# henintsoa98/srsRAN_4G

Hardware: AMD Instinct MI355X
Metric: turbo-decoded info Mbps + PDSCH subframes/s, 20 MHz 64QAM, 1/2/4/8 GPU (higher is better)
Workload: dtype int16; 1 GPU; tdec all 188 LTE CB sizes x 1024 CBs, 8 half-its, rm_turbo SB layout; cb_sizes=188, parallelism=cb-sharded x1, tdec16=auto

## Files before the change

include/srsran_tdec.h:

```cpp
#ifndef SRSRAN_AMD_TDEC_H
#define SRSRAN_AMD_TDEC_H

#include <stdbool.h>
#include <stdint.h>

#ifdef __cplusplus
extern "C" {
#endif

#ifndef SRSRAN_SUCCESS
#define SRSRAN_SUCCESS 0
#define SRSRAN_ERROR -1
#define SRSRAN_ERROR_INVALID_INPUTS -2
#endif

#define SRSRAN_TCOD_RATE 3
#define SRSRAN_TCOD_TOTALTAIL 12
#define SRSRAN_TCOD_MAX_LEN_CB 6144
#define SRSRAN_TDEC_EXPECT_INPUT_SB 1
#define SRSRAN_NOF_TC_CB_SIZES 188

typedef enum {
  SRSRAN_TDEC_AUTO = 0,
  SRSRAN_TDEC_GENERIC,
  SRSRAN_TDEC_SSE,
  SRSRAN_TDEC_SSE_WINDOW,
  SRSRAN_TDEC_NEON_WINDOW,
  SRSRAN_TDEC_AVX_WINDOW,
  SRSRAN_TDEC_SSE8_WINDOW,
  SRSRAN_TDEC_AVX8_WINDOW,
  SRSRAN_TDEC_NOF_IMP
} srsran_tdec_impl_type_t;

typedef struct {
  uint32_t                max_long_cb;
  bool                    force_not_sb;
  srsran_tdec_impl_type_t dec_type;
  uint32_t                current_long_cb;
  int                     current_cbidx;
  int                     n_iter;
  void*                   gpu;
} srsran_tdec_t;

int srsran_tdec_init(srsran_tdec_t* h, uint32_t max_long_cb);
int srsran_tdec_init_manual(srsran_tdec_t* h, uint32_t max_long_cb, srsran_tdec_impl_type_t dec_type);
void srsran_tdec_free(srsran_tdec_t* h);
void srsran_tdec_force_not_sb(srsran_tdec_t* h);
int srsran_tdec_new_cb(srsran_tdec_t* h, uint32_t long_cb);
int srsran_tdec_get_nof_iterations(srsran_tdec_t* h);
uint32_t srsran_tdec_autoimp_get_subblocks(uint32_t long_cb);
uint32_t srsran_tdec_autoimp_get_subblocks_8bit(uint32_t long_cb);
void srsran_tdec_iteration(srsran_tdec_t* h, int16_t* input, uint8_t* output);
int srsran_tdec_run_all(srsran_tdec_t* h, int16_t* input, uint8_t* output, uint32_t nof_iterations, uint32_t long_cb);
void srsran_tdec_iteration_8bit(srsran_tdec_t* h, int8_t* input, uint8_t* output);
int  srsran_tdec_run_all_8bit(srsran_tdec_t* h, int8_t* input, uint8_t* output, uint32_t nof_iterations, uint32_t long_cb);

int srsran_tdec_gpu_run_batch_8bit(uint32_t      long_cb,
                                   const int8_t* d_input,
                                   uint32_t      in_stride,
                                   int           layout_sb,
                                   uint8_t*      d_output,
                                   uint32_t      nof_cb,
                                   uint32_t      nof_iterations,
                                   void*         stream);

int srsran_tdec_run_all_batch(srsran_tdec_t* h,
                              const int16_t* input,
                              uint32_t       in_stride,
                              uint8_t*       output,
                              uint32_t       nof_cb,
                              uint32_t       nof_iterations,
                              uint32_t       long_cb);

int srsran_tdec_gpu_run_batch(uint32_t       long_cb,
                              const int16_t* d_input,
                              uint32_t       in_stride,
                              int            layout_sb,
                              uint8_t*       d_output,
                              uint32_t       nof_cb,
                              uint32_t       nof_iterations,
                              void*          stream);

int srsran_tdec_gpu_run_multi(uint32_t              nof_groups,
                              const uint32_t*       long_cb,
                              const int16_t* const* d_input,
                              const uint32_t*       in_stride,
                              int                   layout_sb,
                              uint8_t* const*       d_output,
                              const uint32_t*       nof_cb,
                              uint32_t              nof_iterations,
                              void*                 stream);

int srsran_tdec_gpu_available(void);

const char* srsran_tdec_gpu_kernel_name(uint32_t long_cb);

const char* srsran_tdec_gpu_kernel_name_batch(uint32_t long_cb, uint32_t nof_cb);

const char* srsran_tdec_gpu_last_kernel(void);

void     srsran_tdec_gpu_set_pair_threshold(uint32_t nof_cb);
uint32_t srsran_tdec_gpu_get_pair_threshold(void);
void     srsran_tdec_gpu_set_class_single_threshold(uint32_t nof_subblocks, uint32_t nof_cb);
uint32_t srsran_tdec_gpu_get_class_single_threshold(uint32_t nof_subblocks);
void     srsran_tdec_gpu_set_single_threshold(uint32_t nof_cb);
uint32_t srsran_tdec_gpu_get_single_threshold(void);
void     srsran_tdec_gpu_set_generic_single_threshold(uint32_t nof_cb);
void     srsran_tdec_gpu_set_w8_max_k(uint32_t k);
uint32_t srsran_tdec_gpu_get_w8_max_k(void);
void     srsran_tdec_gpu_set_w8_fused_max_k(uint32_t k);
uint32_t srsran_tdec_gpu_get_w8_fused_max_k(void);
uint32_t srsran_tdec_gpu_get_generic_single_threshold(void);

#ifdef __cplusplus
}
#endif
#endif
```

srsran_4g_amd/csrc/tdec_api.cpp:

```cpp
#include <hip/hip_runtime.h>

#include <cstdio>
#include <cstdlib>
#include <algorithm>
#include <cstring>
#include <map>
#include <tuple>
#include <mutex>
#include <vector>

#include "../../include/srsran_tdec.h"
#include "stage_copy.h"
#include "devkey.h"
#include "tdec_kernel.h"
#include "tdec8bit_kernel.h"

using namespace srsran_amd;

namespace {

const uint16_t kCbSizes[SRSRAN_NOF_TC_CB_SIZES] = {
    40,   48,   56,   64,   72,   80,   88,   96,   104,  112,  120,  128,  136,  144,  152,  160,  168,  176,  184,
    192,  200,  208,  216,  224,  232,  240,  248,  256,  264,  272,  280,  288,  296,  304,  312,  320,  328,  336,
    344,  352,  360,  368,  376,  384,  392,  400,  408,  416,  424,  432,  440,  448,  456,  464,  472,  480,  488,
    496,  504,  512,  528,  544,  560,  576,  592,  608,  624,  640,  656,  672,  688,  704,  720,  736,  752,  768,
    784,  800,  816,  832,  848,  864,  880,  896,  912,  928,  944,  960,  976,  992,  1008, 1024, 1056, 1088, 1120,
    1152, 1184, 1216, 1248, 1280, 1312, 1344, 1376, 1408, 1440, 1472, 1504, 1536, 1568, 1600, 1632, 1664, 1696, 1728,
    1760, 1792, 1824, 1856, 1888, 1920, 1952, 1984, 2016, 2048, 2112, 2176, 2240, 2304, 2368, 2432, 2496, 2560, 2624,
    2688, 2752, 2816, 2880, 2944, 3008, 3072, 3136, 3200, 3264, 3328, 3392, 3456, 3520, 3584, 3648, 3712, 3776, 3840,
    3904, 3968, 4032, 4096, 4160, 4224, 4288, 4352, 4416, 4480, 4544, 4608, 4672, 4736, 4800, 4864, 4928, 4992, 5056,
    5120, 5184, 5248, 5312, 5376, 5440, 5504, 5568, 5632, 5696, 5760, 5824, 5888, 5952, 6016, 6080, 6144};

const uint16_t kF1[SRSRAN_NOF_TC_CB_SIZES] = {
    3,   7,   19,  7,   7,   11,  5,   11,  7,   41,  103, 15,  9,   17,  9,   21,  101, 21,  57, 23,  13,
    27,  11,  27,  85,  29,  33,  15,  17,  33,  103, 19,  19,  37,  19,  21,  21,  115, 193, 21, 133, 81,
    45,  23,  243, 151, 155, 25,  51,  47,  91,  29,  29,  247, 29,  89,  91,  157, 55,  31,  17, 35,  227,
    65,  19,  37,  41,  39,  185, 43,  21,  155, 79,  139, 23,  217, 25,  17,  127, 25,  239, 17, 137, 215,
    29,  15,  147, 29,  59,  65,  55,  31,  17,  171, 67,  35,  19,  39,  19,  199, 21,  211, 21, 43,  149,
    45,  49,  71,  13,  17,  25,  183, 55,  127, 27,  29,  29,  57,  45,  31,  59,  185, 113, 31, 17,  171,
    209, 253, 367, 265, 181, 39,  27,  127, 143, 43,  29,  45,  157, 47,  13,  111, 443, 51,  51, 451, 257,
    57,  313, 271, 179, 331, 363, 375, 127, 31,  33,  43,  33,  477, 35,  233, 357, 337, 37,  71, 71,  37,
    39,  127, 39,  39,  31,  113, 41,  251, 43,  21,  43,  45,  45,  161, 89,  323, 47,  23,  47, 263};
const uint16_t kF2[SRSRAN_NOF_TC_CB_SIZES] = {
    10,  12,  42,  16,  18,  20,  22,  24,  26,  84,  90,  32,  34,  108, 38,  120, 84,  44,  46,  48,  50,
    52,  36,  56,  58,  60,  62,  32,  198, 68,  210, 36,  74,  76,  78,  120, 82,  84,  86,  44,  90,  46,
    94,  48,  98,  40,  102, 52,  106, 72,  110, 168, 114, 58,  118, 180, 122, 62,  84,  64,  66,  68,  420,
    96,  74,  76,  234, 80,  82,  252, 86,  44,  120, 92,  94,  48,  98,  80,  102, 52,  106, 48,  110, 112,
    114, 58,  118, 60,  122, 124, 84,  64,  66,  204, 140, 72,  74,  76,  78,  240, 82,  252, 86,  88,  60,
    92,  846, 48,  28,  80,  102, 104, 954, 96,  110, 112, 114, 116, 354, 120, 610, 124, 420, 64,  66,  136,
    420, 216, 444, 456, 468, 80,  164, 504, 172, 88,  300, 92,  188, 96,  28,  240, 204, 104, 212, 192, 220,
    336, 228, 232, 236, 120, 244, 248, 168, 64,  130, 264, 134, 408, 138, 280, 142, 480, 146, 444, 120, 152,
    462, 234, 158, 80,  96,  902, 166, 336, 170, 86,  174, 176, 178, 120, 182, 184, 186, 94,  190, 480};

int cb_index(uint32_t K)
{
  for (int i = 0; i < SRSRAN_NOF_TC_CB_SIZES; i++) {
    if (kCbSizes[i] == K) {
      return i;
    }
  }
  return -1;
}

constexpr size_t kMaxLds = 160 * 1024;

struct Config {
  int       nsb;
  TdecArgs  proto;
  uint16_t* d_tfwd = nullptr;
  uint16_t* d_trev = nullptr;
  uint16_t* d_tfwd_nat = nullptr;
  uint16_t* d_trev_nat = nullptr;
};

std::mutex                             g_mu;
std::map<std::tuple<int, uint32_t, int>, Config*> g_cfg;
int                                    g_have_gpu = -1;

bool have_gpu()
{
  if (g_have_gpu < 0) {
    int n = 0;
    g_have_gpu = (hipGetDeviceCount(&n) == hipSuccess && n > 0) ? 1 : 0;
  }
  return g_have_gpu == 1;
}

Config* get_config(uint32_t K, int nsb)
{
  std::lock_guard<std::mutex> lk(g_mu);
  auto key = std::make_tuple(cur_dev(), K, nsb);
  auto it  = g_cfg.find(key);
  if (it != g_cfg.end()) {
    return it->second;
  }
  const int idx = cb_index(K);
  if (idx < 0 || !have_gpu()) {
    return nullptr;
  }
  TdecArgs a{};
  a.K = K;
  if (nsb > 1) {
    if (K % nsb || K / nsb < (uint32_t)TDEC_OVERLAP) {
      return nullptr;
    }
    a.L   = K / nsb;
    a.Ls  = a.L | 1u;
    a.xyw = nsb * a.Ls;
    a.M   = (a.L + TDEC_W - 1) / TDEC_W;
  } else {
    a.L   = K;
    a.Ls  = (K + 3) | 1u;
    a.xyw = a.Ls;
    a.M   = (K + 3 + TDEC_W - 1) / TDEC_W;
  }
  a.magicL  = (uint32_t)(((1ull << 32) + a.L - 1) / a.L);
  a.magicLs = (uint32_t)(((1ull << 32) + a.Ls - 1) / a.Ls);
  if (tdec_lds_bytes(nsb, a.xyw, a.M) > kMaxLds) {
    return nullptr;
  }
  std::vector<uint16_t> fwd(K), rev(K), tf(K), tr(K), tfn(K), trn(K);
  const uint64_t f1 = kF1[idx], f2 = kF2[idx];
  for (uint64_t i = 0; i < K; i++) {
    const uint32_t j = (uint32_t)((f1 * i + f2 * i * i) % K);
    fwd[i]           = (uint16_t)j;
    rev[j]           = (uint16_t)i;
  }
  auto slot = [&](uint32_t n) -> uint16_t {
    return nsb > 1 ? (uint16_t)((n / a.L) * a.Ls + n % a.L) : (uint16_t)n;
  };
  for (uint32_t q = 0; q < K; q++) {
    const uint32_t n = nsb > 1 ? (q % nsb) * a.L + q / nsb : q;
    tf[q]            = slot(fwd[n]);
    tr[q]            = slot(rev[n]);
    tfn[q]           = slot(fwd[q]);
    trn[q]           = slot(rev[q]);
  }
  Config* c = new Config();
  c->nsb    = nsb;
  c->proto  = a;
  auto up = [&](uint16_t** d, const std::vector<uint16_t>& h) {
    return hipMalloc(d, K * sizeof(uint16_t)) == hipSuccess &&
           hipMemcpy(*d, h.data(), K * sizeof(uint16_t), hipMemcpyHostToDevice) == hipSuccess;
  };
  if (!up(&c->d_tfwd, tf) || !up(&c->d_trev, tr) || !up(&c->d_tfwd_nat, tfn) || !up(&c->d_trev_nat, trn)) {
    fprintf(stderr, "[srsran_tdec] device table allocation failed for K=%u\n", K);
    delete c;
    return nullptr;
  }
  g_cfg[key] = c;
  return c;
}

int auto_nsb(uint32_t K)
{
  const uint32_t n = srsran_tdec_autoimp_get_subblocks(K);
  return n ? (int)n : 1;
}

int nsb_for(const srsran_tdec_t* h, uint32_t K)
{
  switch (h->dec_type) {
    case SRSRAN_TDEC_AUTO:
      return auto_nsb(K);
    case SRSRAN_TDEC_GENERIC:
      return 1;
    case SRSRAN_TDEC_SSE_WINDOW:
      return 8;
    case SRSRAN_TDEC_AVX_WINDOW:
      return 16;
    default:
      return -1;
  }
}

struct Ctx {
  hipStream_t stream = nullptr;
  short*      d_in   = nullptr;
  uint8_t*    d_out  = nullptr;
  short*      d_state = nullptr;
  size_t      state_elems = 0;
  short*      d_bin  = nullptr;
  uint8_t*    d_bout = nullptr;
  size_t      bin_elems = 0, bout_bytes = 0;
};

const size_t kMaxIn = 3 * (SRSRAN_TCOD_MAX_LEN_CB + 32) + SRSRAN_TCOD_TOTALTAIL;

int enqueue(const Config* c, const short* d_in, uint32_t in_stride, int layout_sb, uint8_t* d_out, uint32_t ncb,
            int n_start, int n_end, short* d_state, hipStream_t stream)
{
  TdecArgs a  = c->proto;
  a.in        = d_in;
  a.in_stride = in_stride;
  a.layout_sb = (c->nsb > 1) ? layout_sb : 0;
  a.ncb       = ncb;
  a.n_start   = n_start;
  a.n_end     = n_end;
  a.out       = d_out;
  a.tfwd      = c->d_tfwd;
  a.trev      = c->d_trev;
  a.tfwd_nat  = c->d_tfwd_nat;
  a.trev_nat  = c->d_trev_nat;
  a.state     = d_state;
  hipError_t e = tdec_launch(c->nsb, a, stream);
  if (e != hipSuccess) {
    fprintf(stderr, "[srsran_tdec] launch failed: %s\n", hipGetErrorString(e));
    return SRSRAN_ERROR;
  }
  return SRSRAN_SUCCESS;
}

bool grow(void** p, size_t* have, size_t need)
{
  if (*have >= need) {
    return true;
  }
  if (*p) {
    (void)hipFree(*p);
    *p = nullptr;
  }
  if (hipMalloc(p, need) != hipSuccess) {
    *have = 0;
    return false;
  }
  *have = need;
  return true;
}

struct XpowTables {
  const uint32_t* d[2] = {nullptr, nullptr};
};
std::map<int, XpowTables> g_xpow;

const XpowTables* xpow_tables()
{
  std::lock_guard<std::mutex> lk(g_mu);
  const int dev = cur_dev();
  auto      it  = g_xpow.find(dev);
  if (it != g_xpow.end()) {
    return &it->second;
  }
  const int             nm = SRSRAN_TCOD_MAX_LEN_CB / 8 + 1;
  std::vector<uint32_t> h(nm);
  uint32_t*             d[2] = {nullptr, nullptr};
  const uint32_t        poly[2] = {LTE_CRC24A, LTE_CRC24B};
  for (int i = 0; i < 2; i++) {
    crc24_xpow_table(poly[i], h.data(), nm);
    if (hipMalloc(&d[i], nm * sizeof(uint32_t)) != hipSuccess ||
        hipMemcpy(d[i], h.data(), nm * sizeof(uint32_t), hipMemcpyHostToDevice) != hipSuccess) {
      return nullptr;
    }
  }
  XpowTables& t = g_xpow[dev];
  t.d[0]        = d[0];
  t.d[1]        = d[1];
  return &t;
}

std::map<std::pair<int, uint32_t>, const uint16_t*> g_qpp8;

const uint16_t* qpp8_table(uint32_t K, uint32_t nsb, int idx)
{
  std::lock_guard<std::mutex> lk(g_mu);
  const auto                  key = std::make_pair(cur_dev(), K);
  auto                        it  = g_qpp8.find(key);
  if (it != g_qpp8.end()) {
    return it->second;
  }
  const uint64_t        f1 = kF1[idx], f2 = kF2[idx], Ls = K / nsb;
  std::vector<uint16_t> h(K);
  for (uint64_t j = 0; j < K; j++) {
    const uint64_t n  = (j % nsb) * Ls + j / nsb;
    const uint64_t fn = ((f2 * n % K) * n + f1 * n) % K;
    h[j]              = (uint16_t)((fn % Ls) * nsb + fn / Ls);
  }
  uint16_t* d = nullptr;
  if (hipMalloc((void**)&d, K * sizeof(uint16_t)) != hipSuccess ||
      hipMemcpy(d, h.data(), K * sizeof(uint16_t), hipMemcpyHostToDevice) != hipSuccess) {
    hipFree(d);
    return nullptr;
  }
  g_qpp8[key] = d;
  return d;
}

}

namespace srsran_amd {
void qpp_coeffs(uint32_t idx, uint32_t* f1, uint32_t* f2)
{
  *f1 = kF1[idx];
  *f2 = kF2[idx];
}
}

namespace srsran_amd {

int tdec_cb_index(uint32_t K) { return cb_index(K); }

int tdec_sch_enqueue(uint32_t      K,
                     const TdecCb* d_cbs,
                     uint32_t      ncb,
                     uint8_t*      d_out,
                     uint32_t      out_stride,
                     uint8_t*      d_noi,
                     uint8_t*      d_crc_ok,
                     int           n_end,
                     hipStream_t   stream)
{
  if (ncb == 0) {
    return SRSRAN_SUCCESS;
  }
  Config* c = get_config(K, auto_nsb(K));
  const XpowTables* xp = xpow_tables();
  if (!c || !xp) {
    return SRSRAN_ERROR;
  }
  TdecArgs a   = c->proto;
  a.in         = nullptr;
  a.in_stride  = 0;
  a.layout_sb  = c->nsb > 1 ? 1 : 0;
  a.ncb        = ncb;
  a.n_start    = 0;
  a.n_end      = n_end > 0 ? n_end : 1;
  a.out        = d_out;
  a.tfwd       = c->d_tfwd;
  a.trev       = c->d_trev;
  a.tfwd_nat   = c->d_tfwd_nat;
  a.trev_nat   = c->d_trev_nat;
  a.state      = nullptr;
  a.cbs        = d_cbs;
  a.out_stride = out_stride;
  a.noi_out    = d_noi;
  a.crc_ok     = d_crc_ok;
  a.xpow_a     = xp->d[0];
  a.xpow_b     = xp->d[1];
  a.min_iters  = 2;
  hipError_t e = tdec_launch(c->nsb, a, stream);
  if (e != hipSuccess) {
    fprintf(stderr, "[srsran_sch] turbo launch failed: %s\n", hipGetErrorString(e));
    return SRSRAN_ERROR;
  }
  return SRSRAN_SUCCESS;
}

}

namespace {
struct Scratch8 {
  void*       p = nullptr;
  hipStream_t s = nullptr;
  Scratch8(hipStream_t stream, size_t bytes) : s(stream)
  {
    if (hipMallocAsync(&p, bytes, stream) != hipSuccess) {
      p = nullptr;
    }
  }
  ~Scratch8()
  {
    if (p) {
      hipFreeAsync(p, s);
    }
  }
  Scratch8(const Scratch8&)            = delete;
  Scratch8& operator=(const Scratch8&) = delete;
};
}

namespace srsran_amd {
int tdec8_sch_enqueue(uint32_t      K,
                      const TdecCb* d_cbs,
                      uint32_t      ncb,
                      uint8_t*      d_out,
                      uint32_t      out_stride,
                      uint8_t*      d_noi,
                      uint8_t*      d_crc_ok,
                      int           n_end,
                      hipStream_t   stream)
{
  if (ncb == 0) {
    return SRSRAN_SUCCESS;
  }
  const int      idx = cb_index(K);
  const uint32_t nsb = srsran_tdec_autoimp_get_subblocks_8bit(K);
  const XpowTables* xp = xpow_tables();
  if (idx < 0 || (nsb != 16 && nsb != 32) || !xp) {
    return SRSRAN_ERROR;
  }
  Tdec8Args a{};
  a.in         = nullptr;
  a.layout_sb  = 1;
  a.K          = K;
  a.ncb        = ncb;
  a.n_end      = n_end > 0 ? n_end : 1;
  a.out        = d_out;
  a.cbs        = d_cbs;
  a.out_stride = out_stride;
  a.noi_out    = d_noi;
  a.crc_ok     = d_crc_ok;
  a.xpow_a     = xp->d[0];
  a.xpow_b     = xp->d[1];
  a.min_iters  = 2;
  a.qpp        = qpp8_table(K, nsb, idx);
  if (!a.qpp) {
    return SRSRAN_ERROR;
  }
  Scratch8 beta(stream, tdec8bit_beta_bytes((int)nsb, K, ncb));
  a.beta = (uint2*)beta.p;
  if (!a.beta) {
    return SRSRAN_ERROR;
  }
  const hipError_t e = tdec8bit_launch((int)nsb, a, stream);
  tdec_set_last_kernel(nsb == 32 ? "tdec8bit_kernel<32>" : "tdec8bit_kernel<16>");
  if (e != hipSuccess) {
    fprintf(stderr, "[srsran_sch] 8-bit turbo launch failed: %s\n", hipGetErrorString(e));
    return SRSRAN_ERROR;
  }
  return SRSRAN_SUCCESS;
}
}

extern "C" {

uint32_t srsran_tdec_autoimp_get_subblocks(uint32_t long_cb)
{
  if (!(long_cb % 16) && long_cb > 800) {
    return 16;
  }
  if (!(long_cb % 8) && long_cb > 400) {
    return 8;
  }
  return 0;
}

uint32_t srsran_tdec_autoimp_get_subblocks_8bit(uint32_t long_cb)
{
  if (!(long_cb % 32) && long_cb > 2048) {
    return 32;
  }
  if (!(long_cb % 16) && long_cb > 800) {
    return 16;
  }
  if (!(long_cb % 8) && long_cb > 400) {
    return 8;
  }
  return 0;
}

int srsran_tdec_gpu_available(void)
{
  std::lock_guard<std::mutex> lk(g_mu);
  return have_gpu() ? 1 : 0;
}

const char* srsran_tdec_gpu_kernel_name(uint32_t long_cb)
{
  switch (auto_nsb(long_cb)) {
    case 16:
      return "tdec_kernel<16>";
    case 8:
      return "tdec_kernel<8>";
    default:
      return "tdec_kernel<1>";
  }
}

const char* srsran_tdec_gpu_last_kernel(void) { return tdec_last_kernel(); }

void srsran_tdec_gpu_set_pair_threshold(uint32_t nof_cb) { tdec16_set_min_cb(nof_cb); }

uint32_t srsran_tdec_gpu_get_pair_threshold(void) { return tdec16_min_cb(); }

void srsran_tdec_gpu_set_w8_max_k(uint32_t k) { tdecs_set_w8_max_k(k); }

uint32_t srsran_tdec_gpu_get_w8_max_k(void) { return tdecs_w8_max_k(); }

void srsran_tdec_gpu_set_w8_fused_max_k(uint32_t k) { tdecs_set_w8_fused_max_k(k); }

uint32_t srsran_tdec_gpu_get_w8_fused_max_k(void) { return tdecs_w8_fused_max_k(); }



void srsran_tdec_gpu_set_class_single_threshold(uint32_t nof_subblocks, uint32_t nof_cb)
{
  if (nof_subblocks == 16) {
    tdec16s_set_min_cb(nof_cb);
  } else if (nof_subblocks == 8) {
    tdec8s_set_min_cb(nof_cb);
  } else if (nof_subblocks <= 1) {
    tdec1s_set_min_cb(nof_cb);
  }
}

uint32_t srsran_tdec_gpu_get_class_single_threshold(uint32_t nof_subblocks)
{
  return nof_subblocks == 16 ? tdec16s_min_cb() : nof_subblocks == 8 ? tdec8s_min_cb() : tdec1s_min_cb();
}

void srsran_tdec_gpu_set_single_threshold(uint32_t nof_cb)
{
  tdec16s_set_min_cb(nof_cb);
  tdec8s_set_min_cb(nof_cb);
}

uint32_t srsran_tdec_gpu_get_single_threshold(void) { return tdec16s_min_cb(); }

void srsran_tdec_gpu_set_generic_single_threshold(uint32_t nof_cb) { tdec1s_set_min_cb(nof_cb); }

uint32_t srsran_tdec_gpu_get_generic_single_threshold(void) { return tdec1s_min_cb(); }

const char* srsran_tdec_gpu_kernel_name_batch(uint32_t long_cb, uint32_t nof_cb)
{
  const int nsb = auto_nsb(long_cb);
  if (nsb == 16) {
    const int k = tdec16_choice(nof_cb);
    if (k) {
      return k == 2 ? "tdec16s_kernel" : "tdec16_kernel";
    }
  }
  if (nsb == 8 && nof_cb >= tdec8s_min_cb()) {
    return "tdec8s_kernel";
  }
  if (nsb == 1 && nof_cb >= tdec1s_min_cb()) {
    return "tdec1s_kernel";
  }
  return srsran_tdec_gpu_kernel_name(long_cb);
}

int srsran_tdec_init(srsran_tdec_t* h, uint32_t max_long_cb)
{
  return srsran_tdec_init_manual(h, max_long_cb, SRSRAN_TDEC_AUTO);
}

int srsran_tdec_init_manual(srsran_tdec_t* h, uint32_t max_long_cb, srsran_tdec_impl_type_t dec_type)
{
  if (!h) {
    return SRSRAN_ERROR_INVALID_INPUTS;
  }
  memset(h, 0, sizeof(*h));
  if (dec_type != SRSRAN_TDEC_AUTO && dec_type != SRSRAN_TDEC_GENERIC && dec_type != SRSRAN_TDEC_SSE_WINDOW &&
      dec_type != SRSRAN_TDEC_AVX_WINDOW) {
    fprintf(stderr, "[srsran_tdec] decoder %d not supported\n", (int)dec_type);
    return SRSRAN_ERROR;
  }
  if (max_long_cb > SRSRAN_TCOD_MAX_LEN_CB) {
    return SRSRAN_ERROR;
  }
  {
    std::lock_guard<std::mutex> lk(g_mu);
    if (!have_gpu()) {
      fprintf(stderr, "[srsran_tdec] no HIP device available\n");
      return SRSRAN_ERROR;
    }
  }
  Ctx* c = new Ctx();
  if (hipStreamCreateWithFlags(&c->stream, hipStreamNonBlocking) != hipSuccess ||
      hipMalloc(&c->d_in, kMaxIn * sizeof(short)) != hipSuccess ||
      hipMalloc(&c->d_out, SRSRAN_TCOD_MAX_LEN_CB / 8) != hipSuccess) {
    delete c;
    return SRSRAN_ERROR;
  }
  hipMemset(c->d_in, 0, kMaxIn * sizeof(short));
  h->gpu           = c;
  h->max_long_cb   = max_long_cb;
  h->dec_type      = dec_type;
  h->current_cbidx = -1;
  return SRSRAN_SUCCESS;
}

void srsran_tdec_free(srsran_tdec_t* h)
{
  if (!h) {
    return;
  }
  Ctx* c = (Ctx*)h->gpu;
  if (c) {
    if (c->stream) {
      hipStreamSynchronize(c->stream);
      hipStreamDestroy(c->stream);
    }
    hipFree(c->d_in);
    hipFree(c->d_out);
    hipFree(c->d_state);
    hipFree(c->d_bin);
    hipFree(c->d_bout);
    delete c;
  }
  memset(h, 0, sizeof(*h));
}

void srsran_tdec_force_not_sb(srsran_tdec_t* h)
{
  if (h) {
    h->force_not_sb = true;
  }
}

int srsran_tdec_new_cb(srsran_tdec_t* h, uint32_t long_cb)
{
  if (!h || long_cb > h->max_long_cb) {
    fprintf(stderr, "[srsran_tdec] TDEC was initialized for max_long_cb=%d\n", h ? h->max_long_cb : 0);
    return SRSRAN_ERROR;
  }
  h->n_iter          = 0;
  h->current_long_cb = long_cb;
  h->current_cbidx   = cb_index(long_cb);
  if (h->current_cbidx < 0) {
    fprintf(stderr, "[srsran_tdec] Invalid CB length %d\n", long_cb);
    return SRSRAN_ERROR;
  }
  return SRSRAN_SUCCESS;
}

int srsran_tdec_get_nof_iterations(srsran_tdec_t* h) { return h ? h->n_iter : 0; }

static size_t input_len(const srsran_tdec_t* h, const Config* c, uint32_t K)
{
  const bool sb = !h->force_not_sb && c->nsb > 1;
  return sb ? 3 * (K + 32) + 12 : 3 * K + 12;
}

void srsran_tdec_iteration(srsran_tdec_t* h, int16_t* input, uint8_t* output)
{
  if (!h || !h->gpu || h->current_cbidx < 0) {
    fprintf(stderr, "[srsran_tdec] Error CB index not set (call srsran_tdec_new_cb() first\n");
    return;
  }
  Ctx*           ctx = (Ctx*)h->gpu;
  const uint32_t K   = h->current_long_cb;
  Config*        c   = get_config(K, nsb_for(h, K));
  if (!c) {
    fprintf(stderr, "[srsran_tdec] unsupported K=%u\n", K);
    return;
  }
  const size_t st = 2 * (size_t)c->proto.xyw;
  if (!grow((void**)&ctx->d_state, &ctx->state_elems, st * sizeof(short))) {
    return;
  }
  if (h->n_iter == 0) {
    hipMemcpyAsync(ctx->d_in, input, input_len(h, c, K) * sizeof(short), hipMemcpyHostToDevice, ctx->stream);
  }
  if (enqueue(c, ctx->d_in, (uint32_t)kMaxIn, !h->force_not_sb, ctx->d_out, 1, h->n_iter, h->n_iter + 1,
              ctx->d_state, ctx->stream)) {
    return;
  }
  hipMemcpyAsync(output, ctx->d_out, K / 8, hipMemcpyDeviceToHost, ctx->stream);
  hipStreamSynchronize(ctx->stream);
  h->n_iter++;
}

int srsran_tdec_run_all(srsran_tdec_t* h, int16_t* input, uint8_t* output, uint32_t nof_iterations, uint32_t long_cb)
{
  if (srsran_tdec_new_cb(h, long_cb)) {
    return SRSRAN_ERROR;
  }
  int ret = srsran_tdec_run_all_batch(h, input, 0, output, 1, nof_iterations, long_cb);
  if (ret == SRSRAN_SUCCESS) {
    h->n_iter = nof_iterations > 0 ? (int)nof_iterations : 1;
  }
  return ret;
}

int srsran_tdec_run_all_batch(srsran_tdec_t* h,
                              const int16_t* input,
                              uint32_t       in_stride,
                              uint8_t*       output,
                              uint32_t       nof_cb,
                              uint32_t       nof_iterations,
                              uint32_t       long_cb)
{
  if (!h || !h->gpu || !input || !output) {
    return SRSRAN_ERROR_INVALID_INPUTS;
  }
  if (long_cb > h->max_long_cb || cb_index(long_cb) < 0) {
    return SRSRAN_ERROR;
  }
  if (nof_cb == 0) {
    return SRSRAN_SUCCESS;
  }
  Ctx*    ctx = (Ctx*)h->gpu;
  Config* c   = get_config(long_cb, nsb_for(h, long_cb));
  if (!c) {
    return SRSRAN_ERROR;
  }
  const size_t len = input_len(h, c, long_cb);
  if (in_stride == 0) {
    in_stride = (uint32_t)len;
  }
  if (in_stride < len) {
    return SRSRAN_ERROR_INVALID_INPUTS;
  }
  const size_t in_elems  = (size_t)in_stride * (nof_cb - 1) + len;
  const size_t out_bytes = (size_t)nof_cb * (long_cb / 8);
  if (!grow((void**)&ctx->d_bin, &ctx->bin_elems, in_elems * sizeof(short)) ||
      !grow((void**)&ctx->d_bout, &ctx->bout_bytes, out_bytes)) {
    return SRSRAN_ERROR;
  }
  hipMemcpyAsync(ctx->d_bin, input, in_elems * sizeof(short), hipMemcpyHostToDevice, ctx->stream);
  const int n_end = nof_iterations > 0 ? (int)nof_iterations : 1;
  if (enqueue(c, ctx->d_bin, in_stride, !h->force_not_sb, ctx->d_bout, nof_cb, 0, n_end, nullptr, ctx->stream)) {
    return SRSRAN_ERROR;
  }
  hipMemcpyAsync(output, ctx->d_bout, out_bytes, hipMemcpyDeviceToHost, ctx->stream);
  if (hipStreamSynchronize(ctx->stream) != hipSuccess) {
    fprintf(stderr, "[srsran_tdec] decode failed: %s\n", hipGetErrorString(hipGetLastError()));
    return SRSRAN_ERROR;
  }
  return SRSRAN_SUCCESS;
}

int srsran_tdec_gpu_run_batch(uint32_t       long_cb,
                              const int16_t* d_input,
                              uint32_t       in_stride,
                              int            layout_sb,
                              uint8_t*       d_output,
                              uint32_t       nof_cb,
                              uint32_t       nof_iterations,
                              void*          stream)
{
  if (!d_input || !d_output || cb_index(long_cb) < 0) {
    return SRSRAN_ERROR_INVALID_INPUTS;
  }
  Config* c = get_config(long_cb, auto_nsb(long_cb));
  if (!c) {
    return SRSRAN_ERROR;
  }
  const uint32_t len = (layout_sb && c->nsb > 1) ? 3 * (long_cb + 32) + 12 : 3 * long_cb + 12;
  if (in_stride < len) {
    return SRSRAN_ERROR_INVALID_INPUTS;
  }
  const int n_end = nof_iterations > 0 ? (int)nof_iterations : 1;
  return enqueue(c, d_input, in_stride, layout_sb, d_output, nof_cb, 0, n_end, nullptr, (hipStream_t)stream);
}

namespace {
constexpr int kPoolStreams = 4;
struct MultiDesc {
  char*      h_stage = nullptr;
  char*      d_stage = nullptr;
  size_t     cap     = 0;
  hipEvent_t copied  = nullptr;
  bool       used    = false;
};

struct StreamPool {
  int         device = -1;
  hipStream_t s[kPoolStreams];
  hipEvent_t  done[kPoolStreams];
  hipEvent_t  fork;
  hipEvent_t  large_done;
  MultiDesc   md[6];
};
std::mutex               g_pool_mu;
std::vector<StreamPool*> g_pools;

int multi_mode()
{
  static const int m = [] {
    const char* e = getenv("SRSRAN_AMD_TDEC_MULTI");
    return !e ? 0 : !strcmp(e, "priority") ? 1 : !strcmp(e, "serial") ? 2 : 0;
  }();
  return m;
}

StreamPool* get_pool()
{
  int dev = 0;
  if (hipGetDevice(&dev) != hipSuccess) {
    return nullptr;
  }
  std::lock_guard<std::mutex> lk(g_pool_mu);
  for (auto* p : g_pools) {
    if (p->device == dev) {
      return p;
    }
  }
  StreamPool* p = new StreamPool();
  p->device     = dev;
  int lo = 0, hi = 0;
  if (multi_mode() == 1 && hipDeviceGetStreamPriorityRange(&lo, &hi) != hipSuccess) {
    lo = hi = 0;
  }
  for (int i = 0; i < kPoolStreams; i++) {
    if (hipStreamCreateWithPriority(&p->s[i], hipStreamNonBlocking, i == 0 ? hi : lo) != hipSuccess ||
        srsran_amd::ring_event_create(&p->done[i]) != hipSuccess) {
      return nullptr;
    }
  }
  if (srsran_amd::ring_event_create(&p->fork) != hipSuccess || srsran_amd::ring_event_create(&p->large_done) != hipSuccess) {
    return nullptr;
  }
  for (auto& m : p->md) {
    if (srsran_amd::ring_event_create(&m.copied) != hipSuccess) {
      return nullptr;
    }
  }
  g_pools.push_back(p);
  return p;
}

uint32_t gen_cut()
{
  static const uint32_t c = [] {
    const char* e = getenv("SRSRAN_AMD_TDEC_GEN_CUT");
    return e ? (uint32_t)atoi(e) : 0u;
  }();
  return c;
}

uint32_t tdec_midcut()
{
  static const uint32_t c = [] {
    const char* e = getenv("SRSRAN_AMD_TDEC_MIDCUT");
    return e ? (uint32_t)atoi(e) : 3072u;
  }();
  return c;
}
bool tdec_gate()
{
  static const bool g = [] {
    const char* e = getenv("SRSRAN_AMD_TDEC_GATE");
    return e ? atoi(e) != 0 : true;
  }();
  return g;
}

double launch_cost(uint32_t K, uint32_t ncb)
{
  const int    nsb   = auto_nsb(K);
  const double chain = nsb > 1 ? 3.0 * (K / nsb) + 160.0 : 3.0 * (K + 3);
  const double waves = (double)ncb * 4 * nsb / 64.0;
  return chain * (1.0 + waves / 1024.0);
}
}

int srsran_tdec_gpu_run_multi(uint32_t              nof_groups,
                              const uint32_t*       long_cb,
                              const int16_t* const* d_input,
                              const uint32_t*       in_stride,
                              int                   layout_sb,
                              uint8_t* const*       d_output,
                              const uint32_t*       nof_cb,
                              uint32_t              nof_iterations,
                              void*                 stream)
{
  if (nof_groups == 0) {
    return SRSRAN_SUCCESS;
  }
  if (!long_cb || !d_input || !in_stride || !d_output || !nof_cb) {
    return SRSRAN_ERROR_INVALID_INPUTS;
  }
  std::vector<Config*>  cfg(nof_groups);
  std::vector<uint32_t> order(nof_groups);
  for (uint32_t g = 0; g < nof_groups; g++) {
    if (cb_index(long_cb[g]) < 0 || !d_input[g] || !d_output[g]) {
      return SRSRAN_ERROR_INVALID_INPUTS;
    }
    cfg[g] = get_config(long_cb[g], auto_nsb(long_cb[g]));
    if (!cfg[g]) {
      return SRSRAN_ERROR;
    }
    const uint32_t len = (layout_sb && cfg[g]->nsb > 1) ? 3 * (long_cb[g] + 32) + 12 : 3 * long_cb[g] + 12;
    if (in_stride[g] < len) {
      return SRSRAN_ERROR_INVALID_INPUTS;
    }
    order[g] = g;
  }
  std::sort(order.begin(), order.end(), [&](uint32_t a, uint32_t b) {
    return launch_cost(long_cb[a], nof_cb[a]) > launch_cost(long_cb[b], nof_cb[b]);
  });
  StreamPool* p = get_pool();
  if (!p) {
    return SRSRAN_ERROR;
  }
  hipStream_t user = (hipStream_t)stream;
  if (hipEventRecord(p->fork, user) != hipSuccess) {
    return SRSRAN_ERROR;
  }
  for (int i = 0; i < kPoolStreams; i++) {
    hipStreamWaitEvent(p->s[i], p->fork, 0);
  }
  const int n_end = nof_iterations > 0 ? (int)nof_iterations : 1;
  int       ret   = SRSRAN_SUCCESS;
  const int      cls_nsb[6] = {16, 16, 16, 8, 1, 1};
  const int      cls_st[6]  = {0, 0, 1, 2, 3, 3};
  const uint32_t midcut     = tdec_midcut();
  bool           gated      = false;
  bool           mid_run    = false;
  for (int ci = 0; ci < 6 && ret == SRSRAN_SUCCESS; ci++) {
    if (ci == 1 && hipEventRecord(p->large_done, p->s[0]) != hipSuccess) {
      ret = SRSRAN_ERROR;
      break;
    }
    gated = ci >= 2 && mid_run && tdec_gate() && multi_mode() != 2;
    std::vector<uint32_t> gs;
    uint32_t              cls_cb = 0;
    for (uint32_t i = 0; i < nof_groups; i++) {
      if (cfg[order[i]]->nsb == cls_nsb[ci] && nof_cb[order[i]] > 0) {
        gs.push_back(order[i]);
        cls_cb += nof_cb[order[i]];
      }
    }
    if (gs.empty()) {
      continue;
    }
    const int kind = cls_nsb[ci] == 1               ? (cls_cb >= tdec1s_min_cb() ? 2 : 0)
                     : !layout_sb                   ? 0
                     : cls_nsb[ci] == 16            ? tdec16_choice(cls_cb)
                                                    : (cls_cb >= tdec8s_min_cb() ? 2 : 0);
    const uint32_t cut = std::max(tdecs_w8_max_k(), tdecs_w8_fused_max_k());
    if (cls_nsb[ci] == 16 && kind == 2) {
      const uint32_t lo = ci == 0 ? std::max(cut, midcut) : ci == 1 ? cut : 0;
      const uint32_t hi = ci == 0 ? UINT32_MAX : ci == 1 ? std::max(cut, midcut) : cut;
      gs.erase(std::remove_if(gs.begin(), gs.end(),
                              [&](uint32_t g) { return !(cfg[g]->proto.K > lo && cfg[g]->proto.K <= hi); }),
               gs.end());
    } else if (ci == 1 || ci == 2) {
      gs.clear();
    } else if (ci >= 4 && kind == 0 && gen_cut() > 0) {
      const bool small = ci == 5;
      gs.erase(std::remove_if(gs.begin(), gs.end(), [&](uint32_t g) { return (cfg[g]->proto.K <= gen_cut()) != small; }),
               gs.end());
    } else if (ci == 5) {
      gs.clear();
    }
    if (gs.empty()) {
      continue;
    }
    mid_run        = mid_run || ci == 1;
    hipStream_t st = p->s[multi_mode() == 2 ? 0 : cls_st[ci]];
    if (gated && st != p->s[0] && hipStreamWaitEvent(st, p->large_done, 0) != hipSuccess) {
      ret = SRSRAN_ERROR;
      break;
    }
    if (gs.size() == 1) {
      const uint32_t g = gs[0];
      ret = enqueue(cfg[g], d_input[g], in_stride[g], layout_sb, d_output[g], nof_cb[g], 0, n_end, nullptr, st);
      continue;
    }
    const int  nsbc = cls_nsb[ci];
    uint32_t   kmax = 0;
    for (uint32_t g : gs) {
      kmax = std::max(kmax, cfg[g]->proto.K);
    }
    const bool w8  = kind == 2 && nsbc > 1 && kmax <= (nsbc == 16 ? cut : tdecs_w8_max_k());
    const int  cpw  = kind == 2   ? (nsbc == 16 ? tdecs16::cpw() : nsbc == 8 ? tdecs8::cpw() : tdecs1::cpw())
                      : kind == 1 ? tdec16_cpw()
                                  : tdec_cpw(nsbc);
    const size_t   n     = gs.size();
    const size_t   abyte = n * sizeof(TdecArgs);
    const size_t   need  = abyte + n * sizeof(uint32_t);
    MultiDesc&     m     = p->md[ci];
    if (m.used) {
      hipEventSynchronize(m.copied);
    }
    if (need > m.cap) {
      hipStreamSynchronize(st);
      hipHostFree(m.h_stage);
      hipFree(m.d_stage);
      m.h_stage = m.d_stage = nullptr;
      m.cap                 = 0;
      if (hipHostMalloc((void**)&m.h_stage, 2 * need) != hipSuccess || hipMalloc((void**)&m.d_stage, 2 * need) != hipSuccess) {
        return SRSRAN_ERROR;
      }
      m.cap = 2 * need;
    }
    TdecArgs* ha    = reinterpret_cast<TdecArgs*>(m.h_stage);
    uint32_t* hf    = reinterpret_cast<uint32_t*>(m.h_stage + abyte);
    uint32_t  nblk  = 0;
    size_t    lds   = 0;
    for (size_t k = 0; k < n; k++) {
      const uint32_t g = gs[k];
      const Config*  c = cfg[g];
      TdecArgs       a = c->proto;
      a.in             = d_input[g];
      a.in_stride      = in_stride[g];
      a.layout_sb      = c->nsb > 1 ? layout_sb : 0;
      a.ncb            = nof_cb[g];
      a.n_start        = 0;
      a.n_end          = n_end;
      a.out            = d_output[g];
      a.tfwd           = c->d_tfwd;
      a.trev           = c->d_trev;
      a.tfwd_nat       = c->d_tfwd_nat;
      a.trev_nat       = c->d_trev_nat;
      a.state          = nullptr;
      ha[k]            = a;
      hf[k]            = nblk;
      nblk += (nof_cb[g] + cpw - 1) / cpw;
      lds = std::max(lds, kind == 2   ? (nsbc == 16  ? (w8 ? tdecs16w8::lds_bytes(a) : tdecs16::lds_bytes(a))
                                         : nsbc == 8 ? (w8 ? tdecs8w8::lds_bytes(a) : tdecs8::lds_bytes(a))
                                                     : tdecs1::lds_bytes(a))
                          : kind == 1 ? tdec16_lds_bytes(a)
                                      : tdec_lds_bytes(c->nsb, a.xyw, a.M));
    }
    if (hipMemcpyAsync(m.d_stage, m.h_stage, need, hipMemcpyHostToDevice, st) != hipSuccess) {
      return SRSRAN_ERROR;
    }
    hipEventRecord(m.copied, st);
    m.used = true;
    const TdecArgs* dg = reinterpret_cast<const TdecArgs*>(m.d_stage);
    const uint32_t* df = reinterpret_cast<const uint32_t*>(m.d_stage + abyte);
    if ((kind == 2   ? (nsbc == 16  ? (w8 ? tdecs16w8::multi_launch(dg, df, (int)n, nblk, lds, st)
                                          : tdecs16::multi_launch(dg, df, (int)n, nblk, lds, st))
                        : nsbc == 8 ? (w8 ? tdecs8w8::multi_launch(dg, df, (int)n, nblk, lds, st)
                                          : tdecs8::multi_launch(dg, df, (int)n, nblk, lds, st))
                                    : tdecs1::multi_launch(dg, df, (int)n, nblk, lds, st))
         : kind == 1 ? tdec16_multi_launch(dg, df, (int)n, nblk, lds, st)
                     : tdec_multi_launch(cls_nsb[ci], dg, df, (int)n, nblk, lds, st)) != hipSuccess) {
      ret = SRSRAN_ERROR;
    }
  }
  for (int i = 0; i < kPoolStreams; i++) {
    hipEventRecord(p->done[i], p->s[i]);
    hipStreamWaitEvent(user, p->done[i], 0);
  }
  return ret;
}

#ifdef TDECS_STAMPS
int srsran_tdec_gpu_debug_set_stamps(void* d_buf)
{
  using namespace srsran_amd;
  return tdecs16::set_stamps(d_buf) == hipSuccess && tdecs8::set_stamps(d_buf) == hipSuccess &&
                 tdecs16w8::set_stamps(d_buf) == hipSuccess && tdecs8w8::set_stamps(d_buf) == hipSuccess
             ? SRSRAN_SUCCESS
             : SRSRAN_ERROR;
}
#endif


int srsran_tdec_gpu_run_batch_8bit(uint32_t      long_cb,
                                   const int8_t* d_input,
                                   uint32_t      in_stride,
                                   int           layout_sb,
                                   uint8_t*      d_output,
                                   uint32_t      nof_cb,
                                   uint32_t      nof_iterations,
                                   void*         stream)
{
  using namespace srsran_amd;
  const int idx = cb_index(long_cb);
  if (!d_input || !d_output || idx < 0) {
    return SRSRAN_ERROR_INVALID_INPUTS;
  }
  if (nof_cb == 0) {
    return SRSRAN_SUCCESS;
  }
  hipStream_t    s     = (hipStream_t)stream;
  const uint32_t nsb8  = srsran_tdec_autoimp_get_subblocks_8bit(long_cb);
  const bool     sb    = layout_sb && nsb8 > 0;
  const uint32_t len   = sb ? 3 * (long_cb + 32) + 12 : 3 * long_cb + 12;
  const int      n_end = nof_iterations > 0 ? (int)nof_iterations : 1;
  if (in_stride < len) {
    return SRSRAN_ERROR_INVALID_INPUTS;
  }
  if (nsb8 == 16 || nsb8 == 32) {
    Tdec8Args a{};
    a.in        = d_input;
    a.in_stride = in_stride;
    a.layout_sb = sb ? 1 : 0;
    a.K         = long_cb;
    a.ncb       = nof_cb;
    a.n_end     = n_end;
    a.out       = d_output;
    a.qpp       = qpp8_table(long_cb, nsb8, idx);
    if (!a.qpp) {
      return SRSRAN_ERROR;
    }
    Scratch8 beta(s, tdec8bit_beta_bytes((int)nsb8, long_cb, nof_cb));
    if (!beta.p) {
      return SRSRAN_ERROR;
    }
    a.beta           = (uint2*)beta.p;
    const hipError_t e = tdec8bit_launch((int)nsb8, a, s);
    tdec_set_last_kernel(nsb8 == 32 ? "tdec8bit_kernel<32>" : "tdec8bit_kernel<16>");
    return e == hipSuccess ? SRSRAN_SUCCESS : SRSRAN_ERROR;
  }
  Scratch8 wbuf(s, (size_t)nof_cb * len * sizeof(short));
  short*   wide = (short*)wbuf.p;
  if (!wide) {
    return SRSRAN_ERROR;
  }
  return tdec8bit_widen(d_input, in_stride, wide, len, nof_cb, s) == hipSuccess
             ? srsran_tdec_gpu_run_batch(long_cb, wide, len, sb ? 1 : 0, d_output, nof_cb, nof_iterations, stream)
             : SRSRAN_ERROR;
}

int srsran_tdec_run_all_8bit(srsran_tdec_t* h, int8_t* input, uint8_t* output, uint32_t nof_iterations, uint32_t long_cb)
{
  if (!h || !h->gpu || !input || !output) {
    return SRSRAN_ERROR_INVALID_INPUTS;
  }
  if (srsran_tdec_new_cb(h, long_cb)) {
    return SRSRAN_ERROR;
  }
  const uint32_t nsb8 = srsran_tdec_autoimp_get_subblocks_8bit(long_cb);
  if (h->dec_type != SRSRAN_TDEC_AUTO || nsb8 < 16) {
    Config* c = get_config(long_cb, nsb_for(h, long_cb));
    if (!c) {
      return SRSRAN_ERROR;
    }
    const size_t         n = input_len(h, c, long_cb);
    std::vector<int16_t> wide(n);
    for (size_t i = 0; i < n; i++) {
      wide[i] = input[i];
    }
    return srsran_tdec_run_all(h, wide.data(), output, nof_iterations, long_cb);
  }
  Ctx*           ctx = (Ctx*)h->gpu;
  const bool     sb  = !h->force_not_sb;
  const uint32_t len = sb ? 3 * (long_cb + 32) + 12 : 3 * long_cb + 12;
  if (!grow((void**)&ctx->d_bin, &ctx->bin_elems, len) || !grow((void**)&ctx->d_bout, &ctx->bout_bytes, long_cb / 8)) {
    return SRSRAN_ERROR;
  }
  hipMemcpyAsync(ctx->d_bin, input, len, hipMemcpyHostToDevice, ctx->stream);
  int ret = srsran_tdec_gpu_run_batch_8bit(long_cb, (const int8_t*)ctx->d_bin, len, sb ? 1 : 0, ctx->d_bout, 1,
                                           nof_iterations, ctx->stream);
  if (ret != SRSRAN_SUCCESS) {
    return ret;
  }
  hipMemcpyAsync(output, ctx->d_bout, long_cb / 8, hipMemcpyDeviceToHost, ctx->stream);
  if (hipStreamSynchronize(ctx->stream) != hipSuccess) {
    fprintf(stderr, "[srsran_tdec] 8-bit decode failed: %s\n", hipGetErrorString(hipGetLastError()));
    return SRSRAN_ERROR;
  }
  h->n_iter = nof_iterations > 0 ? (int)nof_iterations : 1;
  return SRSRAN_SUCCESS;
}

void srsran_tdec_iteration_8bit(srsran_tdec_t* h, int8_t* input, uint8_t* output)
{
  if (!h || !h->gpu || h->current_cbidx < 0) {
    fprintf(stderr, "[srsran_tdec] Error CB index not set (call srsran_tdec_new_cb() first\n");
    return;
  }
  const int n = h->n_iter + 1;
  if (srsran_tdec_run_all_8bit(h, input, output, (uint32_t)n, h->current_long_cb) == SRSRAN_SUCCESS) {
    h->n_iter = n;
  }
}

}
```

srsran_4g_amd/csrc/tdec_kernel.h:

```cpp
#ifndef SRSRAN_AMD_TDEC_KERNEL_H
#define SRSRAN_AMD_TDEC_KERNEL_H
#include <hip/hip_runtime.h>
#include <stddef.h>
#include <stdint.h>

namespace srsran_amd {

static constexpr int TDEC_W       = 32;
static constexpr int TDEC_OVERLAP = 40;

struct TdecCb {
  const short*   in;
  const uint8_t* skip;
  uint32_t       slot;
  uint32_t       crc_a;
};
static constexpr uint32_t TDEC_PAD_SLOT = 0xffffffffu;
static constexpr uint64_t TDEC_PAIR_SPAN = ((uint64_t)1 << 31) - ((uint64_t)1 << 16);
static constexpr uint32_t TDEC_GROUP     = 8;

struct TdecArgs {
  const short*    in;
  uint32_t        in_stride;
  int             layout_sb;
  uint32_t        K;
  uint32_t        ncb;
  int             n_start;
  int             n_end;
  uint8_t*        out;
  const uint16_t* tfwd;
  const uint16_t* trev;
  const uint16_t* tfwd_nat;
  const uint16_t* trev_nat;
  short*          state;
  uint32_t        L;
  uint32_t        Ls;
  uint32_t        xyw;
  uint32_t        M;
  uint32_t        magicL;
  uint32_t        magicLs;
  const struct TdecCb* cbs;
  uint32_t        out_stride;
  uint8_t*        noi_out;
  uint8_t*        crc_ok;
  const uint32_t* xpow_a;
  const uint32_t* xpow_b;
  int             min_iters;
};

static constexpr uint32_t LTE_CRC24A = 0x1864CFB;
static constexpr uint32_t LTE_CRC24B = 0x1800063;

hipError_t tdec_launch(int nsb, const TdecArgs& a, hipStream_t stream);
hipError_t tdec_multi_launch(int nsb, const TdecArgs* d_groups, const uint32_t* d_first, int ngroups,
                             uint32_t nblocks, size_t lds, hipStream_t stream);
int        tdec_cpw(int nsb);

bool       tdec16_eligible(int nsb, const TdecArgs& a);
bool       tdec16_pays(uint32_t ncb);
void       tdec16_set_min_cb(uint32_t n);
uint32_t   tdec16_min_cb();
hipError_t tdec16_launch(const TdecArgs& a, hipStream_t stream);
hipError_t tdec16_multi_launch(const TdecArgs* d_groups, const uint32_t* d_first, int ngroups, uint32_t nblocks,
                               size_t lds, hipStream_t stream);
size_t     tdec16_lds_bytes(const TdecArgs& a);
int        tdec16_cpw();
#define SRSRAN_TDECS_API(ns)                                                                               \
  namespace ns {                                                                                           \
  hipError_t launch(const TdecArgs& a, hipStream_t stream);                                                \
  hipError_t multi_launch(const TdecArgs* d_groups, const uint32_t* d_first, int ngroups, uint32_t nblocks, \
                          size_t lds, hipStream_t stream);                                                 \
  size_t     lds_bytes(const TdecArgs& a);                                                                 \
  int        cpw();                                                                                        \
  }
SRSRAN_TDECS_API(tdecs16)
SRSRAN_TDECS_API(tdecs8)
SRSRAN_TDECS_API(tdecs16w8)
SRSRAN_TDECS_API(tdecs8w8)
SRSRAN_TDECS_API(tdecs1)
#undef SRSRAN_TDECS_API
#ifdef TDECS_STAMPS
namespace tdecs16 { hipError_t set_stamps(void* d_buf); }
namespace tdecs8 { hipError_t set_stamps(void* d_buf); }
namespace tdecs16w8 { hipError_t set_stamps(void* d_buf); }
namespace tdecs8w8 { hipError_t set_stamps(void* d_buf); }
#endif
bool       tdec8s_eligible(int nsb, const TdecArgs& a);
bool       tdec1s_eligible(int nsb, const TdecArgs& a);
void       tdecs_set_w8_max_k(uint32_t k);
void       tdecs_set_w8_fused_max_k(uint32_t k);
uint32_t   tdecs_w8_fused_max_k();
uint32_t   tdecs_w8_max_k();
void       tdec8s_set_min_cb(uint32_t n);
uint32_t   tdec8s_min_cb();
void       tdec1s_set_min_cb(uint32_t n);
uint32_t   tdec1s_min_cb();
void       tdec16s_set_min_cb(uint32_t n);
uint32_t   tdec16s_min_cb();
int        tdec16_choice(uint32_t ncb);
size_t     tdec_lds_bytes(int nsb, int xyw, int M);
void crc24_xpow_table(uint32_t poly, uint32_t* out, int nm);

int tdec_sch_enqueue(uint32_t      K,
                     const TdecCb* d_cbs,
                     uint32_t      ncb,
                     uint8_t*      d_out,
                     uint32_t      out_stride,
                     uint8_t*      d_noi,
                     uint8_t*      d_crc_ok,
                     int           n_end,
                     hipStream_t   stream);
int tdec8_sch_enqueue(uint32_t K, const TdecCb* d_cbs, uint32_t ncb, uint8_t* d_out, uint32_t out_stride,
                      uint8_t* d_noi, uint8_t* d_crc_ok, int n_end, hipStream_t stream);
uint32_t tdec_pair_cbs(const TdecCb* src, uint32_t n, size_t dst_group_start, void* dst_vec);
const char* tdec_last_kernel();
void        tdec_set_last_kernel(const char* name);
int tdec_cb_index(uint32_t K);

}
#endif
```

srsran_4g_amd/csrc/tdec_kernel.hip:

```cpp
#include <hip/hip_runtime.h>
#include <algorithm>
#include <vector>
#include <stdint.h>

#include "crc24_dev.h"
#include "tdec_kernel.h"
#include "stage_timing.h"

namespace srsran_amd {

typedef short v2s __attribute__((ext_vector_type(2)));

static constexpr int W        = TDEC_W;
static constexpr int OVERLAP  = TDEC_OVERLAP;
static constexpr short NEGINF = -10000;

__device__ __forceinline__ v2s u2v(uint32_t u) { return __builtin_bit_cast(v2s, u); }
__device__ __forceinline__ uint32_t v2u(v2s v) { return __builtin_bit_cast(uint32_t, v); }

template <bool SAT>
__device__ __forceinline__ v2s padd(v2s a, v2s b)
{
  if constexpr (SAT) {
    return __builtin_elementwise_add_sat(a, b);
  } else {
    return a + b;
  }
}
template <bool SAT>
__device__ __forceinline__ v2s psub(v2s a, v2s b)
{
  if constexpr (SAT) {
    return __builtin_elementwise_sub_sat(a, b);
  } else {
    return a - b;
  }
}
__device__ __forceinline__ v2s pmax(v2s a, v2s b) { return __builtin_elementwise_max(a, b); }
__device__ __forceinline__ v2s lo2(v2s a) { return __builtin_shufflevector(a, a, 0, 0); }
__device__ __forceinline__ v2s hi2(v2s a) { return __builtin_shufflevector(a, a, 1, 1); }
__device__ __forceinline__ v2s swp(v2s a) { return __builtin_shufflevector(a, a, 1, 0); }
__device__ __forceinline__ v2s perm(v2s hi_src, v2s lo_src, uint32_t sel)
{
  return u2v(__builtin_amdgcn_perm(v2u(hi_src), v2u(lo_src), sel));
}
#define QP(a, b, c, d) ((a) | ((b) << 2) | ((c) << 4) | ((d) << 6))
template <int CTRL>
__device__ __forceinline__ v2s dpp(v2s a)
{
  return u2v((uint32_t)__builtin_amdgcn_mov_dpp((int)v2u(a), CTRL, 0xf, 0xf, false));
}

struct LaneSel {
  uint32_t rb;
  uint32_t c0, c1;
  uint32_t gb1, gb2, ga0, ga1;
};

__device__ __forceinline__ LaneSel lane_sel(int j)
{
  LaneSel s;
  const int h = j & 1;
  s.rb        = h ? 0x07060302u : 0x05040100u;
  s.c0        = j < 2 ? 0x07060100u : 0x05040302u;
  s.c1        = j < 2 ? 0x05040302u : 0x07060100u;
  const uint32_t b1[4] = {0x05040c0cu, 0x03020100u, 0x01000302u, 0x0c0c0504u};
  const uint32_t b2[4] = {0x0c0c0504u, 0x01000302u, 0x03020100u, 0x05040c0cu};
  s.gb1                = j == 0 ? b1[0] : (j == 1 ? b1[1] : (j == 2 ? b1[2] : b1[3]));
  s.gb2                = j == 0 ? b2[0] : (j == 1 ? b2[1] : (j == 2 ? b2[2] : b2[3]));
  s.ga0                = h ? 0x0c0c0302u : 0x03020c0cu;
  s.ga1                = h ? 0x05040100u : 0x01000504u;
  return s;
}

template <bool SAT>
__device__ __forceinline__ v2s beta_step(v2s P, v2s xy_in, const LaneSel& ls)
{
  const v2s xys = padd<SAT>(xy_in, swp(xy_in));
  const v2s g1  = perm(xys, xy_in, ls.gb1);
  const v2s t1  = dpp<QP(0, 0, 1, 1)>(P);
  const v2s t2  = dpp<QP(2, 2, 3, 3)>(P);
  const v2s r   = perm(t2, t1, ls.rb);
  return pmax(padd<SAT>(lo2(r), g1), padd<SAT>(hi2(r), swp(g1)));
}

template <bool SAT>
__device__ __forceinline__ void alpha_cand(v2s P, v2s xy_in, const LaneSel& ls, v2s& c0, v2s& c1)
{
  const v2s xys = padd<SAT>(xy_in, swp(xy_in));
  const v2s ga  = perm(xys, xy_in, ls.ga0);
  const v2s gb  = perm(xys, xy_in, ls.ga1);
  const v2s u   = dpp<QP(0, 2, 0, 2)>(P);
  const v2s v   = dpp<QP(1, 3, 1, 3)>(P);
  c0            = padd<SAT>(perm(v, u, ls.c0), ga);
  c1            = padd<SAT>(perm(v, u, ls.c1), gb);
}

template <bool SAT>
__device__ __forceinline__ short llr_out(v2s B, v2s c0, v2s c1)
{
  const v2s m0 = padd<SAT>(B, c0);
  const v2s m1 = padd<SAT>(B, c1);
  v2s q        = pmax(perm(m1, m0, 0x05040100u), perm(m1, m0, 0x07060302u));
  q            = pmax(q, dpp<QP(1, 0, 3, 2)>(q));
  q            = pmax(q, dpp<QP(2, 3, 0, 1)>(q));
  const v2s d  = psub<SAT>(swp(q), q);
  return d.x;
}

template <bool SAT>
__device__ __forceinline__ v2s norm(v2s P)
{
  return psub<SAT>(P, lo2(dpp<QP(0, 0, 0, 0)>(P)));
}

__device__ __forceinline__ v2s init_known(int j) { return j == 0 ? v2s{0, NEGINF} : v2s{NEGINF, NEGINF}; }

__device__ __forceinline__ v2s trellis_pair(const short* xt, const short* yt, int j)
{
  short o[8] = {0, NEGINF, NEGINF, NEGINF, NEGINF, NEGINF, NEGINF, NEGINF};
#pragma unroll
  for (int t = 2; t >= 0; t--) {
    const short x = xt[t], y = yt[t], xy = (short)(x + y);
    short n[8];
    n[0] = max(o[0], (short)(o[4] + xy));
    n[1] = max((short)(o[0] + xy), o[4]);
    n[2] = max((short)(o[1] + x), (short)(o[5] + y));
    n[3] = max((short)(o[1] + y), (short)(o[5] + x));
    n[4] = max((short)(o[2] + y), (short)(o[6] + x));
    n[5] = max((short)(o[2] + x), (short)(o[6] + y));
    n[6] = max((short)(o[3] + xy), o[7]);
    n[7] = max(o[3], (short)(o[7] + xy));
#pragma unroll
    for (int i = 0; i < 8; i++) {
      o[i] = n[i];
    }
  }
  v2s r;
  r.x = j == 0 ? o[0] : (j == 1 ? o[2] : (j == 2 ? o[4] : o[6]));
  r.y = j == 0 ? o[1] : (j == 1 ? o[3] : (j == 2 ? o[5] : o[7]));
  return r;
}

template <int NSB>
struct Geo {
  static constexpr bool SAT   = NSB > 1;
  static constexpr int  G     = 4 * NSB;
  static constexpr int  CPW   = 64 / G;
  static constexpr int  KMAX  = NSB == 16 ? 6144 : (NSB == 8 ? 800 : 400);
  static constexpr int  NPL   = (KMAX + G - 1) / G;
};

struct Smem {
  uint32_t* xy;
  short*    aux;
  uint32_t* ck;
};

template <int NSB>
__device__ __forceinline__ bool beta_norm_at(int p, int K)
{
  if constexpr (NSB > 1) {
    return (p % 2) == 0 && p != 0;
  } else {
    return (p % 4) == 0 && p < K;
  }
}
template <int NSB>
__device__ __forceinline__ bool alpha_norm_at(int t)
{
  if constexpr (NSB > 1) {
    return (t % 2) == 0 && t != 0;
  } else {
    return ((t + 1) % 4) == 0;
  }
}


template <int NSB, bool FULL>
__device__ __forceinline__ v2s beta_window(v2s P, const uint32_t* xy, int p0, int p1, int m, bool store_ck, int K,
                                           uint32_t* ck, int lane, const LaneSel& ls, v2s& stored)
{
  constexpr bool SAT = Geo<NSB>::SAT;
  v2s            xw[W];
#pragma unroll
  for (int i = 0; i < W; i++) {
    if (FULL || p0 + i < p1) {
      xw[i] = u2v(xy[p0 + i]);
    }
  }
#pragma unroll
  for (int i = W - 1; i >= 0; i--) {
    if (FULL || p0 + i < p1) {
      P = beta_step<SAT>(P, xw[i], ls);
      if (i == 0) {
        stored = P;
        if (store_ck) {
          ck[(m - 1) * 64 + lane] = v2u(P);
        }
      }
      if (beta_norm_at<NSB>(p0 + i, K)) {
        P = norm<SAT>(P);
      }
    }
  }
  return P;
}

template <int NSB>
__device__ __forceinline__ v2s alpha_fw_window(v2s P, const uint32_t* xy, int t0, int ma, uint32_t* ck, int lane,
                                               const LaneSel& ls)
{
  constexpr bool SAT = Geo<NSB>::SAT;
  v2s            xw[W];
#pragma unroll
  for (int i = 0; i < W; i++) {
    xw[i] = u2v(xy[t0 + i]);
  }
  ck[ma * 64 + lane] = v2u(P);
#pragma unroll
  for (int i = 0; i < W; i++) {
    v2s c0, c1;
    alpha_cand<SAT>(P, xw[i], ls, c0, c1);
    P = pmax(c0, c1);
    if (alpha_norm_at<NSB>(t0 + i)) {
      P = norm<SAT>(P);
    }
  }
  return P;
}

template <int NSB, bool FULL>
__device__ __forceinline__ v2s alpha_window(v2s P, const uint32_t* xy, short* xyo, int t0, int c, int ta, int Nb,
                                            int K, v2s ckv, const LaneSel& ls)
{
  constexpr bool SAT = Geo<NSB>::SAT;
  v2s            xw[W];
  v2s            bw[W];
#pragma unroll
  for (int i = 0; i < W; i++) {
    if (FULL || t0 + i < c) {
      xw[i] = u2v(xy[t0 + i]);
    }
  }
  v2s       Pb = ckv;
  const int ic = FULL ? W - 1 : c - t0 - 1;
#pragma unroll
  for (int i = W - 1; i >= 0; i--) {
    if (i == ic) {
      bw[i] = Pb;
      if (c < Nb && beta_norm_at<NSB>(c, K)) {
        Pb = norm<SAT>(Pb);
      }
    } else if (i < ic) {
      Pb    = beta_step<SAT>(Pb, xw[i + 1], ls);
      bw[i] = Pb;
      if (beta_norm_at<NSB>(t0 + 1 + i, K)) {
        Pb = norm<SAT>(Pb);
      }
    }
  }
#pragma unroll
  for (int i = 0; i < W; i++) {
    if (FULL || t0 + i < ta) {
      v2s c0, c1;
      alpha_cand<SAT>(P, xw[i], ls, c0, c1);
      const short o = llr_out<SAT>(bw[i], c0, c1);
      P             = pmax(c0, c1);
      if (alpha_norm_at<NSB>(t0 + i)) {
        P = norm<SAT>(P);
      }
      xyo[2 * (t0 + i)] = o;
    }
  }
  return P;
}

template <int NSB>
__device__ __forceinline__ v2s beta_llr_window(v2s P, v2s& Bst, const uint32_t* xy, short* xyo, int t0, int K,
                                               v2s cka, const LaneSel& ls)
{
  constexpr bool SAT = Geo<NSB>::SAT;
  v2s            xw[W];
  v2s            cw0[W], cw1[W];
#pragma unroll
  for (int i = 0; i < W; i++) {
    xw[i] = u2v(xy[t0 + i]);
  }
  v2s a = cka;
#pragma unroll
  for (int i = 0; i < W; i++) {
    alpha_cand<SAT>(a, xw[i], ls, cw0[i], cw1[i]);
    if (i < W - 1) {
      a = pmax(cw0[i], cw1[i]);
      if (alpha_norm_at<NSB>(t0 + i)) {
        a = norm<SAT>(a);
      }
    }
  }
#pragma unroll
  for (int i = W - 1; i >= 0; i--) {
    xyo[2 * (t0 + i)] = llr_out<SAT>(Bst, cw0[i], cw1[i]);
    P                 = beta_step<SAT>(P, xw[i], ls);
    Bst               = P;
    if (beta_norm_at<NSB>(t0 + i, K)) {
      P = norm<SAT>(P);
    }
  }
  return P;
}

template <int NSB>
__device__ __forceinline__ void map_decode(const Smem& sm, int base, int wave, int lane, int j, int s, int K, int L, int Nb, int La,
                           int M, const short* xt, const short* yt)
{
  constexpr bool SAT = Geo<NSB>::SAT;
  const LaneSel  ls  = lane_sel(j);
  const uint32_t* xy = sm.xy + base;
  short*          xyo = reinterpret_cast<short*>(sm.xy + base);
  uint32_t*       ck  = sm.ck;
  const int       Mb  = M;
  const int       Ma  = (La + W - 1) / W;
  const int       h   = max(1, min((Nb + W) / (2 * W), La / W));

  if (wave == 0) {
    v2s P = init_known(j);
    if constexpr (NSB > 1) {
      P = v2s{NEGINF, NEGINF};
#pragma unroll
      for (int k = 0; k < OVERLAP; k++) {
        v2s c0, c1;
        alpha_cand<SAT>(P, u2v(xy[L - OVERLAP + k]), ls, c0, c1);
        P = pmax(c0, c1);
        if (alpha_norm_at<NSB>(k)) {
          P = norm<SAT>(P);
        }
      }
      const v2s prv = u2v((uint32_t)__shfl_up((int)v2u(P), 4, 64));
      P             = (s == 0) ? init_known(j) : prv;
    }
    for (int ma = 0; ma < h; ma++) {
      P = alpha_fw_window<NSB>(P, xy, ma * W, ma, ck, lane, ls);
    }
    __syncthreads();
    for (int ma = h; ma < Ma; ma++) {
      const int t0  = ma * W;
      const v2s ckb = u2v(ck[ma * 64 + lane]);
      if (t0 + W <= La) {
        P = alpha_window<NSB, true>(P, xy, xyo, t0, t0 + W, t0 + W, Nb, K, ckb, ls);
      } else {
        P = alpha_window<NSB, false>(P, xy, xyo, t0, min(t0 + W, Nb), La, Nb, K, ckb, ls);
      }
    }
  } else {
    v2s P = init_known(j);
    if constexpr (NSB > 1) {
      P = v2s{NEGINF, NEGINF};
#pragma unroll
      for (int k = OVERLAP - 1; k >= 0; k--) {
        P = beta_step<SAT>(P, u2v(xy[k]), ls);
        if (beta_norm_at<NSB>(k, K)) {
          P = norm<SAT>(P);
        }
      }
      const v2s nxt = u2v((uint32_t)__shfl_down((int)v2u(P), 4, 64));
      P             = (s == NSB - 1) ? trellis_pair(xt, yt, j) : nxt;
    }
    ck[(Mb - 1) * 64 + lane] = v2u(P);
    v2s Bst                  = P;
    int mb                   = Mb - 1;
    if (Nb - mb * W < W) {
      P = beta_window<NSB, false>(P, xy, mb * W, Nb, mb, mb > h, K, ck, lane, ls, Bst);
      mb--;
    }
    for (; mb >= h; mb--) {
      P = beta_window<NSB, true>(P, xy, mb * W, mb * W + W, mb, mb > h, K, ck, lane, ls, Bst);
    }
    __syncthreads();
    for (mb = h - 1; mb >= 0; mb--) {
      const v2s cka = u2v(ck[mb * 64 + lane]);
      P             = beta_llr_window<NSB>(P, Bst, xy, xyo, mb * W, K, cka, ls);
    }
  }
}

__device__ __forceinline__ uint32_t pack2(short lo, short hi)
{
  return (uint32_t)(uint16_t)lo | ((uint32_t)(uint16_t)hi << 16);
}

template <int NSB, bool ES>
__device__ __forceinline__ void tdec_body(const TdecArgs& a, int bid)
{
  using Gm                = Geo<NSB>;
  constexpr bool SAT      = Gm::SAT;
  constexpr int  G        = Gm::G;
  constexpr int  G2       = 2 * G;
  constexpr int  LOG_NSB  = NSB == 16 ? 4 : (NSB == 8 ? 3 : 0);
  extern __shared__ __attribute__((aligned(16))) uint32_t smem[];

  const int wave = threadIdx.x >> 6;
  const int lane = threadIdx.x & 63;
  const int cw   = lane / G;
  const int g    = lane % G;
  const int t2   = wave * G + g;
  const int s    = g >> 2;
  const int j    = g & 3;
  const int K    = a.K;
  const int L    = a.L;
  const int Ls   = a.Ls;
  const int XYW  = a.xyw;
  const int M    = a.M;
  const int cb   = bid * Gm::CPW + cw;
  const int cbl  = cb < (int)a.ncb ? cb : (int)a.ncb - 1;
  const bool live = cb < (int)a.ncb && (!ES || a.cbs[cbl].slot != TDEC_PAD_SLOT);
  bool done = ES && (!live || *a.cbs[cbl].skip);

  Smem sm;
  sm.xy  = smem;
  sm.aux = reinterpret_cast<short*>(smem + Gm::CPW * XYW);
  sm.ck  = smem + Gm::CPW * XYW + (Gm::CPW * XYW + 1) / 2;
  uint32_t* red  = sm.ck + M * 64;
  uint32_t* xyc  = sm.xy + cw * XYW;
  short*    xylo = reinterpret_cast<short*>(xyc);
  short*    auxc = sm.aux + cw * XYW;

  auto decide_byte = [&](int b, bool after_dec1) -> uint32_t {
    uint32_t byte = 0;
#pragma unroll
    for (int t = 0; t < 8; t++) {
      const int n = 8 * b + t;
      int       sl;
      if constexpr (NSB > 1) {
        const int sb_ = (int)__umulhi((uint32_t)n, a.magicL);
        sl            = sb_ * Ls + (n - sb_ * L);
      } else {
        sl = n;
      }
      const short v = after_dec1 ? xylo[2 * sl] : xylo[2 * a.trev_nat[n]];
      byte |= (uint32_t)(v > 0) << (7 - t);
    }
    return byte;
  };

  const short* in = ES ? a.cbs[cbl].in : a.in + (size_t)cbl * a.in_stride;
  const bool   sb = a.layout_sb;
  auto qslot = [&](int q) -> int { return NSB > 1 ? (q & (NSB - 1)) * Ls + (q >> LOG_NSB) : q; };
  const short* tail = sb ? in + 3 * (K + 32) : in + 3 * K;
  short st[3], p0t[3], x2t[3], p1t[3];
#pragma unroll
  for (int t = 0; t < 3; t++) {
    st[t]  = tail[2 * t];
    p0t[t] = tail[2 * t + 1];
    x2t[t] = tail[6 + 2 * t];
    p1t[t] = tail[6 + 2 * t + 1];
  }
  const bool      vsb = NSB > 1 && sb;
  const uint16_t* tfq = vsb ? a.tfwd : a.tfwd_nat;
  const uint16_t* trq = vsb ? a.trev : a.trev_nat;
  const int       nch = K / 4;
  auto pslot = [&](int p) -> int {
    if constexpr (NSB > 1) {
      if (vsb) {
        return qslot(p);
      }
      const int sbn = (int)__umulhi((uint32_t)p, a.magicL);
      return sbn * Ls + (p - sbn * L);
    } else {
      return p;
    }
  };
  auto for_chunks = [&](int hh, auto&& fn) {
    constexpr int BATCH = NSB == 8 ? 2 : 4;
    const bool    d1    = (hh & 1) == 0;
    const bool    need_t = hh > 0;
    const uint16_t* tab  = d1 ? trq : tfq;
    for (int c0 = t2; c0 < nch; c0 += BATCH * G2) {
      uint2 w0[BATCH], w1[BATCH], w2[BATCH], tv[BATCH];
#pragma unroll
      for (int i = 0; i < BATCH; i++) {
        const int c = c0 + i * G2;
        if (c < nch) {
          if (vsb) {
            const short* b = in + 4 * c;
            if (d1) {
              w0[i] = *reinterpret_cast<const uint2*>(b);
              w1[i] = *reinterpret_cast<const uint2*>(b + (K + 32));
            } else {
              w2[i] = *reinterpret_cast<const uint2*>(b + 2 * (K + 32));
            }
          } else {
            const uint2* b = reinterpret_cast<const uint2*>(in + 12 * c);
            w0[i]          = b[0];
            w1[i]          = b[1];
            w2[i]          = b[2];
          }
          if (need_t) {
            tv[i] = *reinterpret_cast<const uint2*>(tab + 4 * c);
          }
        }
      }
#pragma unroll
      for (int i = 0; i < BATCH; i++) {
        const int c = c0 + i * G2;
        if (c < nch) {
#pragma unroll
          for (int v = 0; v < 4; v++) {
            short x0, x1, x2;
            if (vsb) {
              const uint32_t d0 = v < 2 ? w0[i].x : w0[i].y;
              const uint32_t d1w = v < 2 ? w1[i].x : w1[i].y;
              const uint32_t d2 = v < 2 ? w2[i].x : w2[i].y;
              x0 = (short)((v & 1) ? (d0 >> 16) : (d0 & 0xffff));
              x1 = (short)((v & 1) ? (d1w >> 16) : (d1w & 0xffff));
              x2 = (short)((v & 1) ? (d2 >> 16) : (d2 & 0xffff));
            } else {
              const uint32_t e[6] = {w0[i].x, w0[i].y, w1[i].x, w1[i].y, w2[i].x, w2[i].y};
              auto el = [&](int k) -> short { return (short)((k & 1) ? (e[k >> 1] >> 16) : (e[k >> 1] & 0xffff)); };
              x0 = el(3 * v);
              x1 = el(3 * v + 1);
              x2 = el(3 * v + 2);
            }
            int t = 0;
            if (need_t) {
              const uint32_t d = v < 2 ? tv[i].x : tv[i].y;
              t                = (int)((v & 1) ? (d >> 16) : (d & 0xffff));
            }
            fn(4 * c + v, x0, x1, x2, t);
          }
        }
      }
    }
  };

  if (a.n_start > 0) {
    const short* se = a.state + (size_t)cbl * 2 * XYW;
    for (int i = t2; i < XYW; i += G2) {
      xylo[2 * i] = se[i];
      auxc[i]     = se[XYW + i];
    }
    __syncthreads();
  }

  const int base = cw * XYW + (NSB > 1 ? s * Ls : 0);
  const int Nb   = NSB > 1 ? L : K + 3;
  const int La   = NSB > 1 ? L : K;

  if constexpr (ES) {
    if (live && done && t2 == 0) {
      const uint32_t slot = a.cbs[cbl].slot;
      a.noi_out[slot]     = 0;
      a.crc_ok[slot]      = 1;
    }
  }
  const int h_end = (ES && __syncthreads_or(!done) == 0) ? a.n_start : a.n_end;
  for (int h = a.n_start; h < h_end; h++) {
    if ((h & 1) == 0) {
      if (h == 0) {
        for_chunks(h, [&](int p, short sx, short p0, short, int) { xyc[pslot(p)] = pack2(sx, p0); });
      } else {
        for_chunks(h, [&](int p, short, short, short, int t) { xylo[2 * pslot(p) + 1] = xylo[2 * t]; });
        __syncthreads();
        for_chunks(h, [&](int p, short sx, short p0, short, int) {
          const int   sl = pslot(p);
          const short a1 = (short)(xylo[2 * sl + 1] - auxc[sl]);
          auxc[sl]       = a1;
          const short x  = SAT ? __builtin_elementwise_add_sat(sx, a1) : (short)(sx + a1);
          xyc[sl]        = pack2(x, p0);
        });
      }
      if constexpr (NSB == 1) {
        if (t2 < 3) {
          xyc[K + t2] = pack2(st[t2], p0t[t2]);
        }
      }
    } else {
      for (int p = t2; p < K; p += G2) {
        const int   sl = pslot(p);
        const short e  = xylo[2 * sl];
        auxc[sl]       = h > 1 ? (short)(e - auxc[sl]) : e;
      }
      __syncthreads();
      for_chunks(h, [&](int p, short, short, short p1, int t) { xyc[pslot(p)] = pack2(auxc[t], p1); });
      if constexpr (NSB == 1) {
        if (t2 < 3) {
          xyc[K + t2] = pack2(x2t[t2], p1t[t2]);
        }
      }
    }
    __syncthreads();

    const bool dec1 = (h & 1) == 0;
    map_decode<NSB>(sm, base, wave, lane, j, s, K, L, Nb, La, M, dec1 ? st : x2t, dec1 ? p0t : p1t);
    __syncthreads();

    if constexpr (ES) {
      if (h + 1 >= a.min_iters) {
        const int nbytes = K / 8;
        const int bpt    = (nbytes + G2 - 1) / G2;
        const int b0     = t2 * bpt;
        const bool     crc_a = a.cbs[cbl].crc_a;
        const uint32_t poly = crc_a ? LTE_CRC24A : LTE_CRC24B;
        uint32_t       crc  = 0;
        const int      b1   = min(b0 + bpt, nbytes);
#pragma unroll 1
        for (int b = b0; b < b1; b++) {
          crc = crc24_byte(crc, decide_byte(b, dec1), poly);
        }
        uint32_t part = b0 < nbytes ? clmul_mod24(crc, (crc_a ? a.xpow_a : a.xpow_b)[nbytes - b1], poly) : 0;
#pragma unroll
        for (int off = 1; off < G; off <<= 1) {
          part ^= (uint32_t)__shfl_xor((int)part, off, 64);
        }
        if (g == 0) {
          red[cw * 2 + wave] = part;
        }
        __syncthreads();
        const bool ok = (red[cw * 2] ^ red[cw * 2 + 1]) == 0;
        if (ok && !done && live) {
          const uint32_t slot = a.cbs[cbl].slot;
          uint8_t*       out  = a.out + (size_t)slot * a.out_stride;
#pragma unroll 1
          for (int b = b0; b < b1; b++) {
            out[b] = (uint8_t)decide_byte(b, dec1);
          }
          if (t2 == 0) {
            a.noi_out[slot] = (uint8_t)(h + 1);
            a.crc_ok[slot]  = 1;
          }
        }
        done = done || ok;
      }
      if (__syncthreads_or(!done) == 0) {
        break;
      }
    }
  }

  const bool last_dec1 = ((a.n_end - 1) & 1) == 0;
  if (live && !done) {
    const int cbm = ES ? (int)a.cbs[cbl].slot : cbl;
    uint8_t*  out = a.out + (size_t)cbm * (ES ? a.out_stride : K / 8);
    for (int b = t2; b < K / 8; b += G2) {
      out[b] = (uint8_t)decide_byte(b, last_dec1);
    }
    if (ES && t2 == 0) {
      a.noi_out[cbm] = (uint8_t)a.n_end;
      a.crc_ok[cbm]  = 0;
    }
    if (a.state) {
      short* se = a.state + (size_t)cbm * 2 * XYW;
      for (int i = t2; i < XYW; i += G2) {
        se[i]       = xylo[2 * i];
        se[XYW + i] = auxc[i];
      }
    }
  }
}

template <int NSB, bool ES>
__global__ __launch_bounds__(128, 2) void tdec_kernel(TdecArgs a)
{
  tdec_body<NSB, ES>(a, blockIdx.x);
}

template <int NSB>
__global__ __launch_bounds__(128, 2) void tdec_multi_kernel(const TdecArgs* __restrict__ groups,
                                                            const uint32_t* __restrict__ first, int ngroups)
{
  const uint32_t b  = blockIdx.x;
  int            lo = 0, hi = ngroups - 1;
  while (lo < hi) {
    const int mid = (lo + hi + 1) >> 1;
    if (first[mid] <= b) {
      lo = mid;
    } else {
      hi = mid - 1;
    }
  }
  const TdecArgs a = groups[lo];
  tdec_body<NSB, false>(a, (int)(b - first[lo]));
}

hipError_t tdec_multi_launch(int nsb, const TdecArgs* d_groups, const uint32_t* d_first, int ngroups,
                             uint32_t nblocks, size_t lds, hipStream_t stream)
{
  StageScope timing_scope(ST_TDEC, stream);
  if (ngroups == 0 || nblocks == 0) {
    return hipSuccess;
  }
  tdec_set_last_kernel(nsb == 16 ? "tdec_multi_kernel<16>" : nsb == 8 ? "tdec_multi_kernel<8>" : "tdec_multi_kernel<1>");
  switch (nsb) {
    case 16:
      hipLaunchKernelGGL(tdec_multi_kernel<16>, dim3(nblocks), dim3(128), lds, stream, d_groups, d_first, ngroups);
      break;
    case 8:
      hipLaunchKernelGGL(tdec_multi_kernel<8>, dim3(nblocks), dim3(128), lds, stream, d_groups, d_first, ngroups);
      break;
    case 1:
      hipLaunchKernelGGL(tdec_multi_kernel<1>, dim3(nblocks), dim3(128), lds, stream, d_groups, d_first, ngroups);
      break;
    default:
      return hipErrorInvalidValue;
  }
  return hipGetLastError();
}

int tdec_cpw(int nsb) { return 64 / (4 * nsb); }

template <int NSB>
static hipError_t launch(const TdecArgs& a, hipStream_t stream)
{
  StageScope timing_scope(ST_TDEC, stream);
  const int    cpw  = Geo<NSB>::CPW;
  const int    grid = (a.ncb + cpw - 1) / cpw;
  const size_t lds  = tdec_lds_bytes(NSB, a.xyw, a.M);
  tdec_set_last_kernel(NSB == 16 ? "tdec_kernel<16>" : NSB == 8 ? "tdec_kernel<8>" : "tdec_kernel<1>");
  if (a.cbs) {
    hipLaunchKernelGGL((tdec_kernel<NSB, true>), dim3(grid), dim3(128), lds, stream, a);
  } else {
    hipLaunchKernelGGL((tdec_kernel<NSB, false>), dim3(grid), dim3(128), lds, stream, a);
  }
  return hipGetLastError();
}

hipError_t tdec_launch(int nsb, const TdecArgs& a, hipStream_t stream)
{
  if (a.ncb == 0) {
    return hipSuccess;
  }
  if (tdec16_eligible(nsb, a)) {
    return tdec16_choice(a.ncb) == 2 ? (a.K <= tdecs_w8_max_k() ? tdecs16w8::launch(a, stream) : tdecs16::launch(a, stream))
                                     : tdec16_launch(a, stream);
  }
  if (tdec8s_eligible(nsb, a)) {
    return a.K <= tdecs_w8_max_k() ? tdecs8w8::launch(a, stream) : tdecs8::launch(a, stream);
  }
  if (tdec1s_eligible(nsb, a)) {
    return tdecs1::launch(a, stream);
  }
  switch (nsb) {
    case 16:
      return launch<16>(a, stream);
    case 8:
      return launch<8>(a, stream);
    case 1:
      return launch<1>(a, stream);
    default:
      return hipErrorInvalidValue;
  }
}

size_t tdec_lds_bytes(int nsb, int xyw, int M)
{
  const int cpw = 64 / (4 * nsb);
  return (size_t)cpw * xyw * 4 + (((size_t)cpw * xyw + 1) / 2) * 4 + (size_t)M * 64 * 4 + (size_t)cpw * 2 * 4;
}

static thread_local const char* t_last_kernel = "";
const char* tdec_last_kernel() { return t_last_kernel; }
void        tdec_set_last_kernel(const char* name) { t_last_kernel = name; }

uint32_t tdec_pair_cbs(const TdecCb* src, uint32_t n, size_t dst_group_start, void* dst_vec)
{
  std::vector<TdecCb>& dst = *static_cast<std::vector<TdecCb>*>(dst_vec);
  uint32_t             pads = 0;
  uintptr_t            lo = 0, hi = 0;
  for (uint32_t i = 0; i < n; i++) {
    const uintptr_t p   = (uintptr_t)src[i].in;
    size_t          pos = (dst.size() - dst_group_start) % TDEC_GROUP;
    if (pos != 0 && (std::max(hi, p) - std::min(lo, p)) >= TDEC_PAIR_SPAN) {
      TdecCb pad = dst.back();
      pad.slot   = TDEC_PAD_SLOT;
      for (; pos < TDEC_GROUP; pos++) {
        dst.push_back(pad);
        pads++;
      }
      pos = 0;
    }
    if (pos == 0) {
      lo = hi = p;
    }
    lo = std::min(lo, p);
    hi = std::max(hi, p);
    dst.push_back(src[i]);
  }
  return pads;
}

void crc24_xpow_table(uint32_t poly, uint32_t* out, int nm)
{
  uint32_t v = 1;
  for (int m = 0; m < nm; m++) {
    out[m] = v;
    for (int k = 0; k < 8; k++) {
      v = (v & 0x800000u) ? ((v << 1) ^ poly) : (v << 1);
      v &= 0xFFFFFFu;
    }
  }
}

}
```

srsran_4g_amd/csrc/tdecs_kernel.hip:

```cpp
#include <hip/hip_runtime.h>
#include <stdint.h>

#include "crc24_dev.h"
#include "stage_timing.h"
#include "tdec_kernel.h"

#ifndef TDECS_NSB
#define TDECS_NSB 16
#endif
#ifndef TDECS_W
#define TDECS_W 16
#endif
#if TDECS_NSB == 16 && TDECS_W == 16
#define TDECS_NS tdecs16
#define TDECS_K(n) tdec16s_##n
#define TDECS_NAME "tdec16s_"
#elif TDECS_NSB == 8 && TDECS_W == 16
#define TDECS_NS tdecs8
#define TDECS_K(n) tdec8s_##n
#define TDECS_NAME "tdec8s_"
#elif TDECS_NSB == 16 && TDECS_W == 8
#define TDECS_NS tdecs16w8
#define TDECS_K(n) tdec16sw8_##n
#define TDECS_NAME "tdec16sw8_"
#elif TDECS_NSB == 8 && TDECS_W == 8
#define TDECS_NS tdecs8w8
#define TDECS_K(n) tdec8sw8_##n
#define TDECS_NAME "tdec8sw8_"
#else
#error "TDECS_NSB must be 16 or 8, TDECS_W 16 or 8"
#endif

namespace srsran_amd {
namespace TDECS_NS {
namespace {

typedef short v2s __attribute__((ext_vector_type(2)));

constexpr int   W    = TDECS_W;
constexpr int   OVL  = TDEC_OVERLAP;
constexpr int   NTR  = (OVL + W - 1) / W;
constexpr int   NSB  = TDECS_NSB;
constexpr short NEG  = -10000;
constexpr int   CPWG = 64 / NSB;
constexpr int   ROWB = 2 * NSB;

#ifdef TDECS_STAMPS
__device__ unsigned long long* g_stamps = nullptr;
#define TDECS_STAMP(k)                                                                               \
  do {                                                                                               \
    if ((threadIdx.x & 63) == 0 && g_stamps && (k) < 64) {                                          \
      g_stamps[((size_t)blockIdx.x * (blockDim.x >> 6) + (threadIdx.x >> 6)) * 64 + (k)] = clock64(); \
    }                                                                                                \
  } while (0)
#else
#define TDECS_STAMP(k) \
  do {                 \
  } while (0)
#endif

__device__ __forceinline__ v2s u2v(uint32_t u) { return __builtin_bit_cast(v2s, u); }
__device__ __forceinline__ uint32_t v2u(v2s v) { return __builtin_bit_cast(uint32_t, v); }
__device__ __forceinline__ v2s padd(v2s a, v2s b) { return __builtin_elementwise_add_sat(a, b); }
__device__ __forceinline__ v2s psub(v2s a, v2s b) { return __builtin_elementwise_sub_sat(a, b); }
__device__ __forceinline__ v2s pmax(v2s a, v2s b) { return __builtin_elementwise_max(a, b); }
__device__ __forceinline__ v2s lo2(v2s a) { return __builtin_shufflevector(a, a, 0, 0); }
__device__ __forceinline__ v2s hi2(v2s a) { return __builtin_shufflevector(a, a, 1, 1); }
__device__ __forceinline__ v2s swp(v2s a) { return __builtin_shufflevector(a, a, 1, 0); }
__device__ __forceinline__ v2s perm(v2s hi_src, v2s lo_src, uint32_t sel)
{
  return u2v(__builtin_amdgcn_perm(v2u(hi_src), v2u(lo_src), sel));
}

struct St {
  v2s a, b, c, d;
};

template <bool BETA>
struct Sel {
  static constexpr uint32_t c = BETA ? 0x01000504u : 0x05040100u;
  static constexpr uint32_t d = BETA ? 0x03020706u : 0x07060302u;
};

struct Bm {
  v2s s, x, y;
};
__device__ __forceinline__ Bm bm(uint32_t xyw)
{
  const v2s xy = u2v(xyw);
  return Bm{padd(xy, swp(xy)), lo2(xy), hi2(xy)};
}

struct Cand {
  v2s c01, c11, c02, c12, c03, c13, c04, c14;
};
__device__ __forceinline__ Cand cand(const St& p, const Bm& m)
{
  Cand c;
  c.c01 = p.a;
  c.c11 = padd(swp(p.a), m.s);
  c.c02 = p.b;
  c.c12 = padd(swp(p.b), m.s);
  c.c03 = padd(p.c, m.y);
  c.c13 = padd(swp(p.c), m.x);
  c.c04 = padd(p.d, m.y);
  c.c14 = padd(swp(p.d), m.x);
  return c;
}
template <bool BETA>
__device__ __forceinline__ St next(const Cand& c)
{
  const v2s o1 = pmax(c.c01, c.c11);
  const v2s o2 = pmax(c.c02, c.c12);
  const v2s o3 = pmax(c.c03, c.c13);
  const v2s o4 = pmax(c.c04, c.c14);
  return St{perm(o3, o1, 0x05040100u), perm(o4, o2, 0x07060302u), perm(o4, o2, Sel<BETA>::c), perm(o3, o1, Sel<BETA>::d)};
}
template <bool BETA>
__device__ __forceinline__ St step(const St& p, uint32_t xyw)
{
  return next<BETA>(cand(p, bm(xyw)));
}

__device__ __forceinline__ short llr(const Cand& c, const St& B)
{
  const v2s b1 = B.a, b2 = swp(B.b), b3 = swp(B.d), b4 = B.c;
  const v2s m0 = pmax(pmax(padd(b1, c.c01), padd(b2, c.c02)), pmax(padd(b3, c.c03), padd(b4, c.c04)));
  const v2s m1 = pmax(pmax(padd(b1, c.c11), padd(b2, c.c12)), pmax(padd(b3, c.c13), padd(b4, c.c14)));
  return psub(pmax(m1, swp(m1)), pmax(m0, swp(m0))).x;
}

__device__ __forceinline__ St norm(const St& p)
{
  const v2s z = lo2(p.a);
  return St{psub(p.a, z), psub(p.b, z), psub(p.c, z), psub(p.d, z)};
}
__device__ __forceinline__ bool norm_at(int k) { return (k & 1) == 0 && k != 0; }
__device__ __forceinline__ bool nrm(int t0, int i) { return (i & 1) == 0 && (i != 0 || t0 != 0); }

__device__ __forceinline__ St neg_state() { return St{v2s{NEG, NEG}, v2s{NEG, NEG}, v2s{NEG, NEG}, v2s{NEG, NEG}}; }
__device__ __forceinline__ St alpha_known() { return St{v2s{0, NEG}, v2s{NEG, NEG}, v2s{NEG, NEG}, v2s{NEG, NEG}}; }

__device__ __forceinline__ St trellis(const short* xt, const short* yt)
{
  short o[8] = {0, NEG, NEG, NEG, NEG, NEG, NEG, NEG};
#pragma unroll
  for (int t = 2; t >= 0; t--) {
    const short x = xt[t], y = yt[t], xy = (short)(x + y);
    short       n[8];
    n[0] = max(o[0], (short)(o[4] + xy));
    n[1] = max((short)(o[0] + xy), o[4]);
    n[2] = max((short)(o[1] + x), (short)(o[5] + y));
    n[3] = max((short)(o[1] + y), (short)(o[5] + x));
    n[4] = max((short)(o[2] + y), (short)(o[6] + x));
    n[5] = max((short)(o[2] + x), (short)(o[6] + y));
    n[6] = max((short)(o[3] + xy), o[7]);
    n[7] = max(o[3], (short)(o[7] + xy));
#pragma unroll
    for (int i = 0; i < 8; i++) {
      o[i] = n[i];
    }
  }
  return St{v2s{o[0], o[4]}, v2s{o[7], o[3]}, v2s{o[2], o[6]}, v2s{o[5], o[1]}};
}

struct Geo {
  int s_dw, ck_dw, bits_dw, cb_dw;
};
__host__ __device__ __forceinline__ Geo geo(int K, int Ls, int M, bool slot)
{
  Geo g;
  g.s_dw    = (NSB * Ls + 1) / 2;
  g.ck_dw   = M * NSB * 4;
  g.bits_dw = slot ? (NSB * Ls + 31) / 32 + 1 : (K / 8 + 3) / 4;
  g.cb_dw   = g.s_dw + g.ck_dw + g.bits_dw + 2;
  return g;
}

struct Raw {
  uint32_t a[W];
  uint16_t slot[W];
  uint32_t b[W];
};

typedef short __attribute__((address_space(3)))* lshort;
typedef __amdgpu_buffer_rsrc_t                   rsrc_t;
__device__ __forceinline__ uint32_t ldb(rsrc_t r, uint32_t voff, uint32_t soff, int imm)
{
  return __builtin_amdgcn_raw_buffer_load_b16(r, voff + imm, soff, 0);
}
__device__ __forceinline__ rsrc_t make_rsrc(const void* p, uint32_t bytes)
{
  const size_t   u  = (size_t)p;
  const uint32_t lo = __builtin_amdgcn_readfirstlane((uint32_t)u);
  const uint32_t hi = __builtin_amdgcn_readfirstlane((uint32_t)(u >> 32));
  return __builtin_amdgcn_make_buffer_rsrc((void*)(((size_t)hi << 32) | lo), 0,
                                           (int)__builtin_amdgcn_readfirstlane(bytes), 0x00020000);
}

struct Lane {
  int       s, K, L, Ls, M, KP;
  uint32_t  magicLs;
  rsrc_t    rin;
  uint32_t  voff;
  rsrc_t    rtf;
  lshort    S;
  lshort    Ssb;
  uint4*    CK;
  uint32_t* BITS;
};

__device__ __forceinline__ void ck_put(const Lane& c, int m, const St& p)
{
  c.CK[m * NSB + c.s] = make_uint4(v2u(p.a), v2u(p.b), v2u(p.c), v2u(p.d));
}
__device__ __forceinline__ St ck_get(const Lane& c, int m)
{
  const uint4 v = c.CK[m * NSB + c.s];
  return St{u2v(v.x), u2v(v.y), u2v(v.z), u2v(v.w)};
}

template <bool D2>
__device__ __forceinline__ void issue(const Lane& c, Raw& r, int t0)
{
  const uint32_t soff = (uint32_t)ROWB * (uint32_t)t0;
  const uint32_t poff = soff + (D2 ? 4u : 2u) * (uint32_t)c.KP;
#ifdef TDECS_FAKELOAD
#pragma unroll
  for (int i = 0; i < W; i++) {
    r.a[i]    = (soff + i) & 0xff;
    r.slot[i] = (uint16_t)((c.s * 37 + t0 + i) & 511);
    r.b[i] = (poff + 3 * i) & 0xff;
  }
#else
#pragma unroll
  for (int i = 0; i < W; i++) {
    if (D2) {
      r.slot[i] = (uint16_t)ldb(c.rtf, 2u * (uint32_t)c.s, soff, ROWB * i);
    } else {
      r.a[i] = ldb(c.rin, c.voff, soff, ROWB * i);
    }
    r.b[i] = ldb(c.rin, c.voff, poff, ROWB * i);
  }
#endif
}

__device__ __forceinline__ uint32_t pin(uint32_t v)
{
  asm volatile("" : "+v"(v));
  return v;
}

__device__ __forceinline__ void set_nat(const Lane& c, int n, short o)
{
  atomicOr(&c.BITS[n >> 5], (uint32_t)(o > 0) << (((n >> 3) & 3) * 8 + 7 - (n & 7)));
}

template <bool D2, int BITS>
__device__ __forceinline__ uint32_t emit(const Lane& c, int k, short o, uint32_t aux, uint32_t xw)
{
  if (D2) {
    const lshort p = (lshort)(size_t)aux;
    *p             = (short)(o - (short)(xw & 0xffffu));
    if (BITS == 2) {
      const uint32_t slot = (uint32_t)(p - c.S);
      atomicOr(&c.BITS[slot >> 5], (uint32_t)(o > 0) << (slot & 31));
    } else if (BITS == 1) {
      const int slot = (int)(p - c.S);
      const int sb   = (int)__umulhi((uint32_t)slot, c.magicLs);
      set_nat(c, slot - sb * (c.Ls - c.L), o);
    }
    return 0;
  }
  c.Ssb[k] = (short)(o - (short)aux);
  if (BITS == 1) {
    set_nat(c, c.s * c.L + k, o);
  }
  return BITS == 2 ? (uint32_t)(o > 0) : 0u;
}

__device__ __forceinline__ void flush_bits(const Lane& c, int t0, uint32_t wbits)
{
  if (wbits) {
    const uint32_t pos = (uint32_t)(c.s * c.Ls + t0);
    const uint64_t v   = (uint64_t)wbits << (pos & 31);
    atomicOr(&c.BITS[pos >> 5], (uint32_t)v);
    if ((uint32_t)(v >> 32)) {
      atomicOr(&c.BITS[(pos >> 5) + 1], (uint32_t)(v >> 32));
    }
  }
}

__device__ __forceinline__ uint32_t nat_byte(const uint32_t* bits, int L, int Ls, uint32_t magicL, int b)
{
  const int      n0  = 8 * b;
  const int      j   = (int)__umulhi((uint32_t)n0, magicL);
  const int      cnt = (j + 1) * L - n0;
  const uint32_t s0  = (uint32_t)(n0 + j * (Ls - L));
  const uint64_t v   = (uint64_t)bits[s0 >> 5] | (uint64_t)bits[(s0 >> 5) + 1] << 32;
  uint32_t       x   = (uint32_t)(v >> (s0 & 31)) & 0x1ffu;
  if (cnt < 8) {
    x = (x & ((1u << cnt) - 1u)) | ((x >> (cnt + Ls - L)) << cnt);
  }
  return __builtin_bitreverse32(x & 0xffu) >> 24;
}

template <bool D2, int BITS, bool FULL>
__device__ __forceinline__ St alpha_llr_window(const Lane& c, St P, int t0, St Pb, const uint32_t* xw,
                                               const uint32_t* aux)
{
  const int L  = c.L;
  const int cc = FULL ? t0 + W : L;
  const int ic = cc - t0 - 1;
  St        bw[W];
#pragma unroll
  for (int i = W - 1; i >= 0; i--) {
    if (FULL ? i == W - 1 : i == ic) {
      bw[i] = Pb;
      if (cc < L && norm_at(cc)) Pb = norm(Pb);
    } else if (FULL || i < ic) {
      Pb    = step<true>(Pb, xw[i + 1]);
      bw[i] = Pb;
      if (FULL ? (i & 1) : norm_at(t0 + 1 + i)) Pb = norm(Pb);
    }
  }
  uint32_t wbits = 0;
#pragma unroll
  for (int i = 0; i < W; i++) {
    if (FULL || t0 + i < L) {
      const Cand  cd = cand(P, bm(xw[i]));
      const short o  = llr(cd, bw[i]);
      P              = next<false>(cd);
      if ((i & 1) == 0) P = norm(P);
      wbits |= emit<D2, BITS>(c, t0 + i, o, aux[i], xw[i]) << i;
    }
  }
  if (BITS == 2 && !D2) {
    flush_bits(c, t0, wbits);
  }
  return P;
}

template <bool FULL>
__device__ __forceinline__ St beta_window(const Lane& c, St P, int t0, bool store, St& Bst, const uint32_t* xw)
{
#pragma unroll
  for (int i = W - 1; i >= 0; i--) {
    if (FULL || t0 + i < c.L) {
      P = step<true>(P, xw[i]);
      if (i == 0) {
        Bst = P;
        if (store) {
          ck_put(c, t0 / W - 1, P);
        }
      }
      if ((i & 1) == 0) P = norm(P);
    }
  }
  return P;
}

template <int IMM>
__device__ __forceinline__ void wait_for()
{
  __builtin_amdgcn_sched_barrier(0);
  __builtin_amdgcn_s_waitcnt(IMM);
  __builtin_amdgcn_sched_barrier(0);
}
__device__ __forceinline__ void wait_vm0() { wait_for<0x0f70>(); }
__device__ __forceinline__ void wait_lgkm0() { wait_for<0xc07f>(); }
__device__ __forceinline__ void wait_all0() { wait_for<0x0070>(); }

__device__ __forceinline__ uint32_t slot_addr(lshort S, uint16_t slot)
{
  uint32_t a;
  asm("v_mad_u32_u16 %0, %1, 2, %2" : "=v"(a) : "v"(__builtin_bit_cast(_Float16, slot)), "v"((uint32_t)(size_t)S));
  return a;
}

template <bool D2>
struct Pipe {
  Raw      g;
  uint32_t dv[W];

  static __device__ __forceinline__ v2s pack(uint32_t lo, uint32_t hi) { return v2s{(short)lo, (short)hi}; }

  __device__ __forceinline__ void load(const Lane& c, int t0)
  {
    issue<D2>(c, g, t0);
    if (!D2) {
#pragma unroll
      for (int i = 0; i < W; i++) {
        dv[i] = (uint16_t)c.Ssb[t0 + i];
      }
    }
  }
  __device__ __forceinline__ void taken(const Lane& c)
  {
    if (D2) {
      wait_vm0();
#pragma unroll
      for (int i = 0; i < W; i++) {
        dv[i] = slot_addr(c.S, g.slot[i]);
      }
    }
  }
  __device__ __forceinline__ void start(const Lane& c, int t0)
  {
    load(c, t0);
    taken(c);
  }
  template <bool LAST = false>
  __device__ __forceinline__ void next(const Lane& c, int tnext, uint32_t* xw, uint32_t* aux)
  {
    if (D2) {
      short    d[W];
      uint32_t pb[W];
#pragma unroll
      for (int i = 0; i < W; i++) {
        aux[i] = dv[i];
        d[i]   = *(lshort)(size_t)aux[i];
        pb[i]  = g.b[i];
      }
      if (!LAST) {
        issue<D2>(c, g, tnext);
      }
      wait_lgkm0();
#pragma unroll
      for (int i = 0; i < W; i++) {
        xw[i] = pin(v2u(pack((uint16_t)d[i], pb[i])));
      }
    } else {
      wait_all0();
#pragma unroll
      for (int i = 0; i < W; i++) {
        xw[i]  = pin(v2u(padd(pack(g.a[i], g.b[i]), u2v(dv[i]))));
        aux[i] = dv[i];
      }
      __builtin_amdgcn_sched_barrier(0);
      if (!LAST) {
        load(c, tnext);
      }
    }
  }
};

template <bool D2, int BITS>
__device__ __forceinline__ void map16s(const Lane& cin, int wave, int st0)
{
  (void)st0;
  Lane c = cin;
  asm volatile("" : "+v"(c.s));
  asm volatile("" : "+v"(c.voff));
  {
    uint32_t ssb = (uint32_t)(size_t)c.Ssb;
    asm volatile("" : "+v"(ssb));
    c.Ssb = (lshort)(size_t)ssb;
  }
  const int L     = c.L;
  const int Mfull = L / W;
  const int Ma    = (L + W - 1) / W;
  const int h     = max(1, min((L + 2 * W - 1) / (2 * W), L / W));
  Pipe<D2>  pp;
  uint32_t  xw[W];
  uint32_t  aux[W];
  if (wave == 0) {
    pp.start(c, L - OVL);
    St P = neg_state();
    TDECS_STAMP(st0);
#pragma unroll
    for (int w = 0; w < NTR; w++) {
      pp.next(c, w < NTR - 1 ? L - OVL + W * (w + 1) : 0, xw, aux);
#pragma unroll
      for (int i = 0; i < (W < OVL - w * W ? W : OVL - w * W); i++) {
        P = step<false>(P, xw[i]);
        if (norm_at(w * W + i)) P = norm(P);
      }
      pp.taken(c);
    }
    TDECS_STAMP(st0 + 1);
    {
      St q;
      q.a = u2v((uint32_t)__shfl_up((int)v2u(P.a), 1, NSB));
      q.b = u2v((uint32_t)__shfl_up((int)v2u(P.b), 1, NSB));
      q.c = u2v((uint32_t)__shfl_up((int)v2u(P.c), 1, NSB));
      q.d = u2v((uint32_t)__shfl_up((int)v2u(P.d), 1, NSB));
      P   = c.s == 0 ? alpha_known() : q;
    }
#pragma unroll 1
    for (int ma = 0; ma < h; ma++) {
      const int t0 = ma * W;
      pp.next(c, t0 + W, xw, aux);
      ck_put(c, ma, P);
#pragma unroll
      for (int i = 0; i < W; i++) {
        P = step<false>(P, xw[i]);
        if (nrm(t0, i)) P = norm(P);
      }
      pp.taken(c);
    }
    TDECS_STAMP(st0 + 2);
    __syncthreads();
    TDECS_STAMP(st0 + 3);
    const int tlast = (Ma - 1) * W;
#pragma unroll 1
    for (int ma = h; ma < Mfull; ma++) {
      pp.next(c, min(ma * W + W, tlast), xw, aux);
      P = alpha_llr_window<D2, BITS, true>(c, P, ma * W, ck_get(c, ma), xw, aux);
      pp.taken(c);
    }
    if (Ma > Mfull) {
      pp.template next<true>(c, 0, xw, aux);
      alpha_llr_window<D2, BITS, false>(c, P, Mfull * W, ck_get(c, Mfull), xw, aux);
    }
    TDECS_STAMP(st0 + 4);
  } else {
    pp.start(c, (NTR - 1) * W);
    St P = neg_state();
    TDECS_STAMP(st0);
#pragma unroll
    for (int w = 0; w < NTR; w++) {
      const int t0 = (NTR - 1 - w) * W;
      pp.next(c, w < NTR - 1 ? t0 - W : (Ma - 1) * W, xw, aux);
#pragma unroll
      for (int i = (W < OVL - t0 ? W : OVL - t0) - 1; i >= 0; i--) {
        P = step<true>(P, xw[i]);
        if (norm_at(t0 + i)) P = norm(P);
      }
      pp.taken(c);
    }
    TDECS_STAMP(st0 + 1);
    {
      St q;
      q.a = u2v((uint32_t)__shfl_down((int)v2u(P.a), 1, NSB));
      q.b = u2v((uint32_t)__shfl_down((int)v2u(P.b), 1, NSB));
      q.c = u2v((uint32_t)__shfl_down((int)v2u(P.c), 1, NSB));
      q.d = u2v((uint32_t)__shfl_down((int)v2u(P.d), 1, NSB));
      if (c.s == NSB - 1) {
        const int tail = 6 * c.KP + (D2 ? 12 : 0);
        short     xt[3], yt[3];
#pragma unroll
        for (int t = 0; t < 3; t++) {
          xt[t] = (short)ldb(c.rin, c.voff - 2 * c.s, tail, 4 * t);
          yt[t] = (short)ldb(c.rin, c.voff - 2 * c.s, tail, 4 * t + 2);
        }
        P = trellis(xt, yt);
      } else {
        P = q;
      }
    }
    const int mtop = Ma - 1;
    ck_put(c, mtop, P);
    St Bst = P;
    if (Ma > Mfull) {
      pp.next(c, (mtop - 1) * W, xw, aux);
      P = beta_window<false>(c, P, mtop * W, mtop > h, Bst, xw);
      pp.taken(c);
    }
#pragma unroll 1
    for (int mb = Mfull - 1; mb >= h; mb--) {
      pp.next(c, mb * W - W, xw, aux);
      P = beta_window<true>(c, P, mb * W, mb > h, Bst, xw);
      pp.taken(c);
    }
    TDECS_STAMP(st0 + 2);
    __syncthreads();
    TDECS_STAMP(st0 + 3);
#pragma unroll 1
    for (int mb = h - 1; mb >= 0; mb--) {
      const int t0 = mb * W;
      pp.next(c, max(t0 - W, 0), xw, aux);
      St Pa = ck_get(c, mb);
      St aw[W];
#pragma unroll
      for (int i = 0; i < W; i++) {
        aw[i] = Pa;
        if (i < W - 1) {
          Pa = step<false>(Pa, xw[i]);
          if (nrm(t0, i)) Pa = norm(Pa);
        }
      }
      uint32_t wbits = 0;
#pragma unroll
      for (int i = W - 1; i >= 0; i--) {
        const short o = llr(cand(aw[i], bm(xw[i])), Bst);
        P             = step<true>(P, xw[i]);
        Bst           = P;
        if (nrm(t0, i)) P = norm(P);
        wbits |= emit<D2, BITS>(c, t0 + i, o, aux[i], xw[i]) << i;
      }
      if (BITS == 2 && !D2) {
        flush_bits(c, t0, wbits);
      }
      pp.taken(c);
    }
    TDECS_STAMP(st0 + 4);
  }
}

}

template <bool ES>
__device__ __forceinline__ void body(const TdecArgs& a, int bid)
{
  constexpr int NT = 128;
  extern __shared__ __attribute__((aligned(16))) uint32_t smem[];
  const int lane = threadIdx.x & 63;
  const int wave = threadIdx.x >> 6;
  const int cbw  = lane / NSB;
  const int s    = lane % NSB;
  const int t2   = wave * NSB + s;
  const int K    = (int)a.K;
  const int L    = (int)a.L;
  const int Ls   = (int)a.Ls;
  const int M    = (L + W - 1) / W;
  const Geo g    = geo(K, Ls, M, ES);
  const int cb   = bid * CPWG + cbw;
  const int cbl  = cb < (int)a.ncb ? cb : (int)a.ncb - 1;
  const bool live = cb < (int)a.ncb && (!ES || a.cbs[cbl].slot != TDEC_PAD_SLOT);
  bool done      = ES && (!live || *a.cbs[cbl].skip);

  uint32_t* base = smem + cbw * g.cb_dw;
  Lane      c;
  c.s       = s;
  c.K       = K;
  c.L       = L;
  c.Ls      = Ls;
  c.M       = M;
  c.KP      = K + 32;
  c.magicLs = a.magicLs;
  const uint32_t magicL = 0xffffffffu / (uint32_t)L + 1u;
  const int cb0 = bid * CPWG;
  size_t    in_lane, in_lo = SIZE_MAX, in_hi = 0;
#pragma unroll
  for (int i = 0; i < CPWG; i++) {
    const int    j = min(cb0 + i, (int)a.ncb - 1);
    const size_t p = ES ? (size_t)a.cbs[j].in : (size_t)(a.in + (size_t)j * a.in_stride);
    in_lo          = min(in_lo, p);
    in_hi          = max(in_hi, p);
  }
  in_lane                 = ES ? (size_t)a.cbs[cbl].in : (size_t)(a.in + (size_t)cbl * a.in_stride);
  const uint32_t cb_bytes = (uint32_t)(3 * c.KP + 12) * 2;
  c.rin  = make_rsrc((const void*)in_lo, (uint32_t)(in_hi - in_lo) + cb_bytes);
  c.voff = (uint32_t)(in_lane - in_lo) + 2 * c.s;
  c.rtf  = make_rsrc(a.tfwd, 2u * (uint32_t)K);
  c.S    = (lshort)(short*)base;
  c.Ssb  = c.S + c.s * Ls;
  c.CK   = reinterpret_cast<uint4*>(base + g.s_dw);
  c.BITS = base + g.s_dw + g.ck_dw;
  uint32_t* RED = c.BITS + g.bits_dw;

  if constexpr (ES) {
    if (live && done && t2 == 0) {
      const uint32_t slot = a.cbs[cbl].slot;
      a.noi_out[slot]     = 0;
      a.crc_ok[slot]      = 1;
    }
  }
  for (int i = threadIdx.x; i < CPWG * g.s_dw; i += NT) {
    smem[(i / g.s_dw) * g.cb_dw + i % g.s_dw] = 0u;
  }
  const int h_end = (ES && __syncthreads_or(!done) == 0) ? 0 : a.n_end;
#ifdef TDECS_STAMPS
  int passed_at = 0, ran = 0;
#endif

#pragma unroll 1
  for (int hi = 0; hi < h_end; hi++) {
    const bool crc_now = ES && hi + 1 >= a.min_iters;
    for (int i = threadIdx.x; i < CPWG * g.bits_dw; i += NT) {
      smem[(i / g.bits_dw) * g.cb_dw + g.s_dw + g.ck_dw + i % g.bits_dw] = 0u;
    }
    __syncthreads();
    const bool    bits = ES ? crc_now : hi + 1 == h_end;
    constexpr int BM   = ES ? 2 : 1;
    if (hi & 1) {
      if (bits) {
        map16s<true, BM>(c, wave, 5 * hi);
      } else {
        map16s<true, 0>(c, wave, 5 * hi);
      }
    } else {
      if (bits) {
        map16s<false, BM>(c, wave, 5 * hi);
      } else {
        map16s<false, 0>(c, wave, 5 * hi);
      }
    }
    __syncthreads();

    if constexpr (ES) {
      if (crc_now) {
        const int      nbytes = K / 8;
        const int      bpt    = (nbytes + 2 * NSB - 1) / (2 * NSB);
        const int      b0     = t2 * bpt;
        const int      b1     = min(b0 + bpt, nbytes);
        const bool     crc_a  = a.cbs[cbl].crc_a;
        const uint32_t poly   = crc_a ? LTE_CRC24A : LTE_CRC24B;
        uint32_t       crc    = 0;
#pragma unroll 1
        for (int b = b0; b < b1; b++) {
          crc = crc24_byte(crc, nat_byte(c.BITS, L, Ls, magicL, b), poly);
        }
        uint32_t part = b0 < nbytes ? clmul_mod24(crc, (crc_a ? a.xpow_a : a.xpow_b)[nbytes - b1], poly) : 0;
#pragma unroll
        for (int off = 1; off < NSB; off <<= 1) {
          part ^= (uint32_t)__shfl_xor((int)part, off, 64);
        }
        if (s == 0) {
          RED[wave] = part;
        }
        __syncthreads();
        const bool ok = (RED[0] ^ RED[1]) == 0;
        if (ok && !done && live) {
          const uint32_t slot = a.cbs[cbl].slot;
          uint8_t*       out  = a.out + (size_t)slot * a.out_stride;
          for (int b = t2; b < nbytes; b += 2 * NSB) {
            out[b] = (uint8_t)nat_byte(c.BITS, L, Ls, magicL, b);
          }
          if (t2 == 0) {
            a.noi_out[slot] = (uint8_t)(hi + 1);
            a.crc_ok[slot]  = 1;
          }
        }
#ifdef TDECS_STAMPS
        if (ok && !done) {
          passed_at = hi + 1;
        }
#endif
        done = done || ok;
      }
#ifdef TDECS_STAMPS
      ran = hi + 1;
#endif
      if (__syncthreads_or(!done) == 0) {
        break;
      }
    }
  }
#ifdef TDECS_STAMPS
  if (ES && g_stamps && t2 == 0 && wave == 0) {
    unsigned long long* st = g_stamps + (size_t)blockIdx.x * (blockDim.x >> 6) * 64;
    st[56 + cbw]           = live ? (unsigned long long)(passed_at ? passed_at : h_end) : 0ull;
    if (cbw == 0) {
      st[63] = (unsigned long long)ran;
    }
  }
#endif

  if (live && !done && h_end > 0) {
    const int      cbm   = ES ? (int)a.cbs[cbl].slot : cbl;
    uint8_t*       out   = a.out + (size_t)cbm * (ES ? a.out_stride : K / 8);
    for (int b = t2; b < K / 8; b += 2 * NSB) {
      out[b] = ES ? (uint8_t)nat_byte(c.BITS, L, Ls, magicL, b) : reinterpret_cast<const uint8_t*>(c.BITS)[b];
    }
    if (ES && t2 == 0) {
      a.noi_out[cbm] = (uint8_t)a.n_end;
      a.crc_ok[cbm]  = 0;
    }
  }
}

template <bool ES>
__global__ __launch_bounds__(128, 1) void TDECS_K(kernel)(TdecArgs a)
{
  body<ES>(a, blockIdx.x);
}

__global__ __launch_bounds__(128, 1) void TDECS_K(multi_kernel)(const TdecArgs* __restrict__ groups,
                                                            const uint32_t* __restrict__ first, int ngroups)
{
  if constexpr (NSB == 16 && W == 16) {
    __builtin_amdgcn_s_setprio(2);
  }
  const uint32_t b  = blockIdx.x;
  int            lo = 0, hi = ngroups - 1;
  while (lo < hi) {
    const int mid = (lo + hi + 1) >> 1;
    if (first[mid] <= b) {
      lo = mid;
    } else {
      hi = mid - 1;
    }
  }
  const TdecArgs a = groups[lo];
  body<false>(a, (int)(b - first[lo]));
}

size_t lds_bytes(const TdecArgs& a)
{
  const Geo g = geo((int)a.K, (int)a.Ls, (int)((a.L + W - 1) / W), a.cbs != nullptr);
  return (size_t)CPWG * g.cb_dw * 4;
}

int cpw() { return CPWG; }

hipError_t launch(const TdecArgs& a, hipStream_t stream)
{
  StageScope timing_scope(ST_TDEC, stream);
  const int    grid = (a.ncb + CPWG - 1) / CPWG;
  const size_t lds  = lds_bytes(a);
  tdec_set_last_kernel(a.cbs ? TDECS_NAME "kernel<true>" : TDECS_NAME "kernel<false>");
  if (a.cbs) {
    hipLaunchKernelGGL((TDECS_K(kernel)<true>), dim3(grid), dim3(128), lds, stream, a);
  } else {
    hipLaunchKernelGGL((TDECS_K(kernel)<false>), dim3(grid), dim3(128), lds, stream, a);
  }
  return hipGetLastError();
}

hipError_t multi_launch(const TdecArgs* d_groups, const uint32_t* d_first, int ngroups, uint32_t nblocks, size_t lds,
                        hipStream_t stream)
{
  StageScope timing_scope(ST_TDEC, stream);
  if (ngroups == 0 || nblocks == 0) {
    return hipSuccess;
  }
  tdec_set_last_kernel(TDECS_NAME "multi_kernel");
  hipLaunchKernelGGL(TDECS_K(multi_kernel), dim3(nblocks), dim3(128), lds, stream, d_groups, d_first, ngroups);
  return hipGetLastError();
}

#ifdef TDECS_STAMPS
hipError_t set_stamps(void* d_buf)
{
  unsigned long long* p = (unsigned long long*)d_buf;
  return hipMemcpyToSymbol(HIP_SYMBOL(g_stamps), &p, sizeof(p));
}
#endif

}
}
```

srsran_4g_amd/tdec.py:

```python
import ctypes
import os

import numpy as np

HERE = os.path.dirname(os.path.abspath(__file__))
LIB_PATH = os.environ.get("SRSRAN_AMD_LIB") or os.path.join(HERE, "lib", "libsrsran_4g_amd.so")

SRSRAN_SUCCESS = 0
SRSRAN_ERROR = -1
SRSRAN_ERROR_INVALID_INPUTS = -2
SRSRAN_TCOD_MAX_LEN_CB = 6144

SRSRAN_TDEC_AUTO = 0
SRSRAN_TDEC_GENERIC = 1
SRSRAN_TDEC_SSE = 2
SRSRAN_TDEC_SSE_WINDOW = 3
SRSRAN_TDEC_NEON_WINDOW = 4
SRSRAN_TDEC_AVX_WINDOW = 5
SRSRAN_TDEC_SSE8_WINDOW = 6
SRSRAN_TDEC_AVX8_WINDOW = 7

CB_SIZES = (
    [40 + 8 * i for i in range(60)]
    + [528 + 16 * i for i in range(32)]
    + [1056 + 32 * i for i in range(32)]
    + [2112 + 64 * i for i in range(64)]
)


class srsran_tdec_t(ctypes.Structure):

    _fields_ = [
        ("max_long_cb", ctypes.c_uint32),
        ("force_not_sb", ctypes.c_bool),
        ("dec_type", ctypes.c_int),
        ("current_long_cb", ctypes.c_uint32),
        ("current_cbidx", ctypes.c_int),
        ("n_iter", ctypes.c_int),
        ("gpu", ctypes.c_void_p),
    ]


_i16p = ctypes.POINTER(ctypes.c_int16)
_u8p = ctypes.POINTER(ctypes.c_uint8)
_lib = None


def load_library():
    global _lib
    if _lib is not None:
        return _lib
    if not os.path.exists(LIB_PATH):
        raise FileNotFoundError(f"{LIB_PATH} missing: run __graft_entry__.build() (make -C srsran_4g_amd/csrc)")
    lib = ctypes.CDLL(LIB_PATH)
    P = ctypes.POINTER(srsran_tdec_t)
    u32 = ctypes.c_uint32
    sig = {
        "srsran_tdec_init": ([P, u32], ctypes.c_int),
        "srsran_tdec_init_manual": ([P, u32, ctypes.c_int], ctypes.c_int),
        "srsran_tdec_free": ([P], None),
        "srsran_tdec_force_not_sb": ([P], None),
        "srsran_tdec_new_cb": ([P, u32], ctypes.c_int),
        "srsran_tdec_get_nof_iterations": ([P], ctypes.c_int),
        "srsran_tdec_autoimp_get_subblocks": ([u32], u32),
        "srsran_tdec_autoimp_get_subblocks_8bit": ([u32], u32),
        "srsran_tdec_iteration": ([P, _i16p, _u8p], None),
        "srsran_tdec_run_all": ([P, _i16p, _u8p, u32, u32], ctypes.c_int),
        "srsran_tdec_iteration_8bit": ([P, ctypes.POINTER(ctypes.c_int8), _u8p], None),
        "srsran_tdec_run_all_8bit": ([P, ctypes.POINTER(ctypes.c_int8), _u8p, u32, u32], ctypes.c_int),
        "srsran_tdec_run_all_batch": ([P, _i16p, u32, _u8p, u32, u32, u32], ctypes.c_int),
        "srsran_tdec_gpu_run_batch": ([u32, ctypes.c_void_p, u32, ctypes.c_int, ctypes.c_void_p, u32, u32,
                                       ctypes.c_void_p], ctypes.c_int),
        "srsran_tdec_gpu_run_batch_8bit": ([u32, ctypes.c_void_p, u32, ctypes.c_int, ctypes.c_void_p, u32, u32,
                                            ctypes.c_void_p], ctypes.c_int),
        "srsran_tdec_gpu_run_multi": ([u32, ctypes.POINTER(u32), ctypes.POINTER(ctypes.c_void_p), ctypes.POINTER(u32),
                                       ctypes.c_int, ctypes.POINTER(ctypes.c_void_p), ctypes.POINTER(u32), u32,
                                       ctypes.c_void_p], ctypes.c_int),
        "srsran_tdec_gpu_available": ([], ctypes.c_int),
        "srsran_tdec_gpu_kernel_name": ([u32], ctypes.c_char_p),
        "srsran_tdec_gpu_kernel_name_batch": ([u32, u32], ctypes.c_char_p),
        "srsran_tdec_gpu_last_kernel": ([], ctypes.c_char_p),
        "srsran_tdec_gpu_set_pair_threshold": ([u32], None),
        "srsran_tdec_gpu_get_pair_threshold": ([], u32),
        "srsran_tdec_gpu_set_single_threshold": ([u32], None),
        "srsran_tdec_gpu_get_single_threshold": ([], u32),
        "srsran_tdec_gpu_set_class_single_threshold": ([u32, u32], None),
        "srsran_tdec_gpu_get_class_single_threshold": ([u32], u32),
        "srsran_tdec_gpu_set_generic_single_threshold": ([u32], None),
        "srsran_tdec_gpu_set_w8_max_k": ([u32], None),
        "srsran_tdec_gpu_get_w8_max_k": ([], u32),
        "srsran_tdec_gpu_set_w8_fused_max_k": ([u32], None),
        "srsran_tdec_gpu_get_w8_fused_max_k": ([], u32),
        "srsran_tdec_gpu_get_generic_single_threshold": ([], u32),
    }
    for name, (args, res) in sig.items():
        f = getattr(lib, name)
        f.argtypes = args
        f.restype = res
    _lib = lib
    return lib


def last_kernel():
    return load_library().srsran_tdec_gpu_last_kernel().decode()


class pair_threshold:

    def __init__(self, nof_cb):
        self.n = nof_cb

    def __enter__(self):
        lib = load_library()
        self.old = lib.srsran_tdec_gpu_get_pair_threshold()
        lib.srsran_tdec_gpu_set_pair_threshold(self.n)
        return self

    def __exit__(self, *exc):
        load_library().srsran_tdec_gpu_set_pair_threshold(self.old)


class w8_max_k(pair_threshold):

    def __enter__(self):
        lib = load_library()
        self.old = lib.srsran_tdec_gpu_get_w8_max_k()
        lib.srsran_tdec_gpu_set_w8_max_k(self.n)
        return self

    def __exit__(self, *exc):
        load_library().srsran_tdec_gpu_set_w8_max_k(self.old)


class w8_fused_max_k(pair_threshold):

    def __enter__(self):
        lib = load_library()
        self.old = lib.srsran_tdec_gpu_get_w8_fused_max_k()
        lib.srsran_tdec_gpu_set_w8_fused_max_k(self.n)
        return self

    def __exit__(self, *exc):
        load_library().srsran_tdec_gpu_set_w8_fused_max_k(self.old)


class class_single_threshold:
    classes = (16, 8)

    def __init__(self, nof_cb, classes=None):
        self.n = nof_cb
        if classes is not None:
            self.classes = tuple(classes)

    def __enter__(self):
        lib = load_library()
        self.old = {c: lib.srsran_tdec_gpu_get_class_single_threshold(c) for c in self.classes}
        for c in self.classes:
            lib.srsran_tdec_gpu_set_class_single_threshold(c, self.n)
        return self

    def __exit__(self, *exc):
        lib = load_library()
        for c, n in self.old.items():
            lib.srsran_tdec_gpu_set_class_single_threshold(c, n)


class single_threshold(class_single_threshold):
    classes = (16, 8)


class generic_single_threshold(class_single_threshold):
    classes = (0,)


def nof_subblocks(K):
    return load_library().srsran_tdec_autoimp_get_subblocks(K)


def input_len(K, layout_sb):
    return 3 * (K + 32) + 12 if (layout_sb and nof_subblocks(K)) else 3 * K + 12


def gpu_available():
    return bool(load_library().srsran_tdec_gpu_available())


class TurboDecoder:

    def __init__(self, max_long_cb=SRSRAN_TCOD_MAX_LEN_CB, dec_type=SRSRAN_TDEC_AUTO):
        self.lib = load_library()
        self.h = srsran_tdec_t()
        rc = self.lib.srsran_tdec_init_manual(ctypes.byref(self.h), max_long_cb, dec_type)
        if rc != SRSRAN_SUCCESS:
            raise RuntimeError(f"srsran_tdec_init_manual failed ({rc}); is a HIP device visible?")

    def free(self):
        if self.h.gpu:
            self.lib.srsran_tdec_free(ctypes.byref(self.h))

    def __del__(self):
        try:
            self.free()
        except Exception:
            pass

    def force_not_sb(self):
        self.lib.srsran_tdec_force_not_sb(ctypes.byref(self.h))

    @property
    def layout_sb(self):
        return not self.h.force_not_sb

    def new_cb(self, K):
        return self.lib.srsran_tdec_new_cb(ctypes.byref(self.h), K)

    def get_nof_iterations(self):
        return self.lib.srsran_tdec_get_nof_iterations(ctypes.byref(self.h))

    def iteration(self, llr):
        llr = np.ascontiguousarray(llr, dtype=np.int16)
        K = self.h.current_long_cb
        out = np.zeros(K // 8, dtype=np.uint8)
        n0 = self.h.n_iter
        self.lib.srsran_tdec_iteration(ctypes.byref(self.h), llr.ctypes.data_as(_i16p), out.ctypes.data_as(_u8p))
        if self.h.n_iter != n0 + 1:
            raise RuntimeError("srsran_tdec_iteration failed")
        return out

    def run_all(self, llr, nof_iterations, K):
        llr = np.ascontiguousarray(llr, dtype=np.int16)
        out = np.zeros(K // 8, dtype=np.uint8)
        rc = self.lib.srsran_tdec_run_all(ctypes.byref(self.h), llr.ctypes.data_as(_i16p),
                                          out.ctypes.data_as(_u8p), nof_iterations, K)
        if rc != SRSRAN_SUCCESS:
            raise RuntimeError(f"srsran_tdec_run_all failed ({rc})")
        return out

    def run_all_8bit(self, llr, nof_iterations, K):
        llr = np.ascontiguousarray(llr, dtype=np.int8)
        out = np.zeros(K // 8, dtype=np.uint8)
        rc = self.lib.srsran_tdec_run_all_8bit(ctypes.byref(self.h), llr.ctypes.data_as(ctypes.POINTER(ctypes.c_int8)),
                                               out.ctypes.data_as(_u8p), nof_iterations, K)
        if rc != SRSRAN_SUCCESS:
            raise RuntimeError(f"srsran_tdec_run_all_8bit failed ({rc})")
        return out

    def iteration_8bit(self, llr):
        llr = np.ascontiguousarray(llr, dtype=np.int8)
        K = self.h.current_long_cb
        out = np.zeros(K // 8, dtype=np.uint8)
        n0 = self.h.n_iter
        self.lib.srsran_tdec_iteration_8bit(ctypes.byref(self.h), llr.ctypes.data_as(ctypes.POINTER(ctypes.c_int8)),
                                            out.ctypes.data_as(_u8p))
        if self.h.n_iter != n0 + 1:
            raise RuntimeError("srsran_tdec_iteration_8bit failed")
        return out

    def run_all_batch(self, llr2d, nof_iterations, K):
        llr2d = np.ascontiguousarray(llr2d, dtype=np.int16)
        n = llr2d.shape[0]
        out = np.zeros((n, K // 8), dtype=np.uint8)
        rc = self.lib.srsran_tdec_run_all_batch(ctypes.byref(self.h), llr2d.ctypes.data_as(_i16p), llr2d.shape[1],
                                                out.ctypes.data_as(_u8p), n, nof_iterations, K)
        if rc != SRSRAN_SUCCESS:
            raise RuntimeError(f"srsran_tdec_run_all_batch failed ({rc})")
        return out


def gpu_run_batch(K, d_in, in_stride, layout_sb, d_out, nof_cb, nof_iterations, stream=None):
    rc = load_library().srsran_tdec_gpu_run_batch(K, d_in, in_stride, int(bool(layout_sb)), d_out, nof_cb,
                                                  nof_iterations, stream)
    if rc != SRSRAN_SUCCESS:
        raise RuntimeError(f"srsran_tdec_gpu_run_batch failed ({rc})")


def gpu_run_batch_8bit(K, d_in, in_stride, layout_sb, d_out, nof_cb, nof_iterations, stream=None):
    rc = load_library().srsran_tdec_gpu_run_batch_8bit(K, d_in, in_stride, int(bool(layout_sb)), d_out, nof_cb,
                                                       nof_iterations, stream)
    if rc != SRSRAN_SUCCESS:
        raise RuntimeError(f"srsran_tdec_gpu_run_batch_8bit failed ({rc})")


def gpu_run_multi(Ks, d_ins, strides, layout_sb, d_outs, ncbs, nof_iterations, stream=None):
    n = len(Ks)
    u32 = ctypes.c_uint32
    vp = ctypes.c_void_p
    rc = load_library().srsran_tdec_gpu_run_multi(
        n, (u32 * n)(*Ks), (vp * n)(*d_ins), (u32 * n)(*strides), int(bool(layout_sb)), (vp * n)(*d_outs),
        (u32 * n)(*ncbs), nof_iterations, stream)
    if rc != SRSRAN_SUCCESS:
        raise RuntimeError(f"srsran_tdec_gpu_run_multi failed ({rc})")
```

Before: 35330 Mbps.

## Add lean 16-subblock tdec kernel variant allowing multiple workgroups per CU

Adds a 'lean' build of the 16-subblock shuffle turbo decoder whose launch bounds allow two waves per SIMD. It recomputes lane-derived addresses on demand to cut register pressure and uses DPP row shifts instead of cross-lane shuffles. Host code finds, per device, the largest code-block sizes whose LDS footprint lets 3 or 4 workgroups share a CU. It routes mid and large K classes to this kernel in the multi-group scheduler, adding a new tier class and moving the gating point. The goal is higher occupancy and latency hiding; the cost is recomputation overhead and possible register spills.

```diff
diff --git a/include/srsran_tdec.h b/include/srsran_tdec.h
--- a/include/srsran_tdec.h
+++ b/include/srsran_tdec.h
@@ -111,6 +111,10 @@
 void     srsran_tdec_gpu_set_w8_fused_max_k(uint32_t k);
 uint32_t srsran_tdec_gpu_get_w8_fused_max_k(void);
 uint32_t srsran_tdec_gpu_get_generic_single_threshold(void);
+void     srsran_tdec_gpu_set_lean(int mode);
+int      srsran_tdec_gpu_get_lean(void);
+void     srsran_tdec_gpu_set_lean_cuts(uint32_t k4, uint32_t k3);
+uint32_t srsran_tdec_gpu_get_lean_cut(uint32_t nof_workgroups);
 
 #ifdef __cplusplus
 }
diff --git a/srsran_4g_amd/csrc/tdec_api.cpp b/srsran_4g_amd/csrc/tdec_api.cpp
--- a/srsran_4g_amd/csrc/tdec_api.cpp
+++ b/srsran_4g_amd/csrc/tdec_api.cpp
@@ -174,6 +174,128 @@
   }
 }
 
+#ifndef TDEC_LEAN_DEFAULT
+#define TDEC_LEAN_DEFAULT 1
+#endif
+#ifndef TDEC_LEAN_FUSED_DEFAULT
+#define TDEC_LEAN_FUSED_DEFAULT false
+#endif
+#ifndef TDEC_LEAN_MID_DEFAULT
+#define TDEC_LEAN_MID_DEFAULT true
+#endif
+
+struct LeanDev {
+  bool     ok = false;
+  uint32_t k4 = 0, k3 = 0;
+  int      cus = 0;
+};
+std::map<int, LeanDev> g_lean;
+int      g_lean_mode = -1;
+uint32_t g_lean_set_k4 = 0, g_lean_set_k3 = 0;
+
+size_t lean_lds(uint32_t K)
+{
+  TdecArgs a{};
+  a.K  = K;
+  a.L  = K / 16;
+  a.Ls = a.L | 1u;
+  return tdecs16l::lds_bytes(a);
+}
+
+LeanDev lean_dev()
+{
+  std::lock_guard<std::mutex> lk(g_mu);
+  const int dev = cur_dev();
+  auto      it  = g_lean.find(dev);
+  if (it != g_lean.end()) {
+    return it->second;
+  }
+  LeanDev d;
+  int     lds_cu = 0;
+  if (have_gpu() && hipDeviceGetAttribute(&lds_cu, hipDeviceAttributeMaxSharedMemoryPerMultiprocessor, dev) == hipSuccess &&
+      hipDeviceGetAttribute(&d.cus, hipDeviceAttributeMultiprocessorCount, dev) == hipSuccess && lds_cu >= 128) {
+    const size_t block = (size_t)lds_cu / 128;
+    auto bound = [&](int n) -> uint32_t {
+      for (int i = SRSRAN_NOF_TC_CB_SIZES - 1; i >= 0 && auto_nsb(kCbSizes[i]) == 16; i--) {
+        const size_t lds = lean_lds(kCbSizes[i]);
+        if ((lds + block - 1) / block * block * (size_t)n <= (size_t)lds_cu && tdecs16l::occupancy(lds) >= n) {
+          return kCbSizes[i];
+        }
+      }
+      return 0;
+    };
+    d.k3 = bound(3);
+    d.k4 = bound(4);
+    d.ok = d.k3 > 0 && d.k4 > 0 && d.cus > 0;
+  }
+  g_lean[dev] = d;
+  return d;
+}
+
+int lean_mode()
+{
+  if (g_lean_mode < 0) {
+    const char* e = getenv("SRSRAN_AMD_TDEC_LEAN");
+    g_lean_mode   = e ? std::min(std::max(atoi(e), 0), 2) : TDEC_LEAN_DEFAULT;
+    if ((e = getenv("SRSRAN_AMD_TDEC_LEAN_K4")) && !g_lean_set_k4) {
+      g_lean_set_k4 = (uint32_t)atoi(e);
+    }
+    if ((e = getenv("SRSRAN_AMD_TDEC_LEAN_K3")) && !g_lean_set_k3) {
+      g_lean_set_k3 = (uint32_t)atoi(e);
+    }
+  }
+  return g_lean_mode;
+}
+
+bool lean_fused_on()
+{
+  static const bool g = [] {
+    const char* e = getenv("SRSRAN_AMD_TDEC_LEAN_FUSED");
+    return e ? atoi(e) != 0 : TDEC_LEAN_FUSED_DEFAULT;
+  }();
+  return g;
+}
+
+bool lean_mid_on()
+{
+  static const bool g = [] {
+    const char* e = getenv("SRSRAN_AMD_TDEC_LEAN_MID");
+    return e ? atoi(e) != 0 : TDEC_LEAN_MID_DEFAULT;
+  }();
+  return g;
+}
+
+struct Lean {
+  int      mode = 0;
+  uint32_t k4 = 0, k3 = 0;
+  int      cus = 0;
+};
+Lean lean_state(int mode)
+{
+  Lean l;
+  if (mode == 0) {
+    return l;
+  }
+  const LeanDev d = lean_dev();
+  if (!d.ok) {
+    return l;
+  }
+  l.mode = mode;
+  l.k3   = g_lean_set_k3 ? std::min(g_lean_set_k3, d.k3) : d.k3;
+  l.k4   = std::min(g_lean_set_k4 ? std::min(g_lean_set_k4, d.k4) : d.k4, l.k3);
+  l.cus  = d.cus;
+  return l;
+}
+
+bool lean_gate_after_tier()
+{
+  static const bool g = [] {
+    const char* e = getenv("SRSRAN_AMD_TDEC_LEAN_GATE");
+    return e ? atoi(e) != 0 : true;
+  }();
+  return g;
+}
+
 struct Ctx {
   hipStream_t stream = nullptr;
   short*      d_in   = nullptr;
@@ -188,7 +310,7 @@
 const size_t kMaxIn = 3 * (SRSRAN_TCOD_MAX_LEN_CB + 32) + SRSRAN_TCOD_TOTALTAIL;
 
 int enqueue(const Config* c, const short* d_in, uint32_t in_stride, int layout_sb, uint8_t* d_out, uint32_t ncb,
-            int n_start, int n_end, short* d_state, hipStream_t stream)
+            int n_start, int n_end, short* d_state, hipStream_t stream, bool lean = false)
 {
   TdecArgs a  = c->proto;
   a.in        = d_in;
@@ -203,7 +325,7 @@
   a.tfwd_nat  = c->d_tfwd_nat;
   a.trev_nat  = c->d_trev_nat;
   a.state     = d_state;
-  hipError_t e = tdec_launch(c->nsb, a, stream);
+  hipError_t e = lean ? tdecs16l::launch(a, stream) : tdec_launch(c->nsb, a, stream);
   if (e != hipSuccess) {
     fprintf(stderr, "[srsran_tdec] launch failed: %s\n", hipGetErrorString(e));
     return SRSRAN_ERROR;
@@ -285,6 +407,14 @@
   return d;
 }
 
+}
+
+namespace srsran_amd {
+bool tdec_lean_single(uint32_t K, uint32_t ncb)
+{
+  const Lean l = lean_state(lean_mode());
+  return l.mode == 2 ? K <= l.k3 : l.mode == 1 && K <= l.k4 && ncb > 2u * 4u * (uint32_t)l.cus;
+}
 }
 
 namespace srsran_amd {
@@ -480,6 +610,22 @@
 
 uint32_t srsran_tdec_gpu_get_w8_fused_max_k(void) { return tdecs_w8_fused_max_k(); }
 
+void srsran_tdec_gpu_set_lean(int mode) { g_lean_mode = std::min(std::max(mode, 0), 2); }
+
+int srsran_tdec_gpu_get_lean(void) { return lean_mode(); }
+
+void srsran_tdec_gpu_set_lean_cuts(uint32_t k4, uint32_t k3)
+{
+  g_lean_set_k4 = k4;
+  g_lean_set_k3 = k3;
+}
+
+uint32_t srsran_tdec_gpu_get_lean_cut(uint32_t nof_workgroups)
+{
+  const Lean l = lean_state(1);
+  return nof_workgroups == 4 ? l.k4 : nof_workgroups == 3 ? l.k3 : 0;
+}
+
 
 
 void srsran_tdec_gpu_set_class_single_threshold(uint32_t nof_subblocks, uint32_t nof_cb)
@@ -516,7 +662,8 @@
   if (nsb == 16) {
     const int k = tdec16_choice(nof_cb);
     if (k) {
-      return k == 2 ? "tdec16s_kernel" : "tdec16_kernel";
+      return k != 2 ? "tdec16_kernel"
+             : long_cb > tdecs_w8_max_k() && tdec_lean_single(long_cb, nof_cb) ? "tdec16sl_kernel" : "tdec16s_kernel";
     }
   }
   if (nsb == 8 && nof_cb >= tdec8s_min_cb()) {
@@ -750,7 +897,7 @@
   hipEvent_t  done[kPoolStreams];
   hipEvent_t  fork;
   hipEvent_t  large_done;
-  MultiDesc   md[6];
+  MultiDesc   md[7];
 };
 std::mutex               g_pool_mu;
 std::vector<StreamPool*> g_pools;
@@ -883,17 +1030,35 @@
   }
   const int n_end = nof_iterations > 0 ? (int)nof_iterations : 1;
   int       ret   = SRSRAN_SUCCESS;
-  const int      cls_nsb[6] = {16, 16, 16, 8, 1, 1};
-  const int      cls_st[6]  = {0, 0, 1, 2, 3, 3};
-  const uint32_t midcut     = tdec_midcut();
-  bool           gated      = false;
-  bool           mid_run    = false;
-  for (int ci = 0; ci < 6 && ret == SRSRAN_SUCCESS; ci++) {
-    if (ci == 1 && hipEventRecord(p->large_done, p->s[0]) != hipSuccess) {
+  enum { E_LARGE, E_TIER3, E_MID, E_W8, E_C8, E_GEN, E_GEN2, E_N };
+  const int      cls_nsb[E_N] = {16, 16, 16, 16, 8, 1, 1};
+  const int      cls_st[E_N]  = {0, 0, 0, 1, 2, 3, 3};
+  const uint32_t midcut       = tdec_midcut();
+  const uint32_t cut          = std::max(tdecs_w8_max_k(), tdecs_w8_fused_max_k());
+  const uint32_t mid_hi       = std::max(cut, midcut);
+  const Lean     lean         = lean_state(lean_mode());
+  auto lean_part = [&](uint32_t lo, uint32_t hi) {
+    uint32_t wgs = 0, kmax = 0;
+    for (uint32_t g = 0; g < nof_groups; g++) {
+      if (cfg[g]->nsb == 16 && nof_cb[g] > 0 && long_cb[g] > lo && long_cb[g] <= hi) {
+        wgs += (nof_cb[g] + tdecs16l::cpw() - 1) / tdecs16l::cpw();
+        kmax = std::max(kmax, long_cb[g]);
+      }
+    }
+    return lean.mode > 0 && wgs > 0 && kmax <= lean.k3 &&
+           (lean.mode == 2 || (lean_fused_on() && wgs > 2u * (uint32_t)lean.cus));
+  };
+  const uint32_t tier_hi  = lean.mode > 0 && lean.k3 > mid_hi && lean_part(mid_hi, lean.k3) ? lean.k3 : mid_hi;
+  const bool     lean_mid = (lean.mode == 2 || lean_mid_on()) && lean_part(cut, mid_hi);
+  const int      gate_at  = tier_hi > mid_hi && !lean_gate_after_tier() ? E_TIER3 : E_MID;
+  bool           gated    = false;
+  bool           mid_run  = false;
+  for (int ci = 0; ci < E_N && ret == SRSRAN_SUCCESS; ci++) {
+    if (ci == gate_at && hipEventRecord(p->large_done, p->s[0]) != hipSuccess) {
       ret = SRSRAN_ERROR;
       break;
     }
-    gated = ci >= 2 && mid_run && tdec_gate() && multi_mode() != 2;
+    gated = ci >= E_W8 && mid_run && tdec_gate() && multi_mode() != 2;
     std::vector<uint32_t> gs;
     uint32_t              cls_cb = 0;
     for (uint32_t i = 0; i < nof_groups; i++) {
@@ -909,26 +1074,26 @@
                      : !layout_sb                   ? 0
                      : cls_nsb[ci] == 16            ? tdec16_choice(cls_cb)
                                                     : (cls_cb >= tdec8s_min_cb() ? 2 : 0);
-    const uint32_t cut = std::max(tdecs_w8_max_k(), tdecs_w8_fused_max_k());
     if (cls_nsb[ci] == 16 && kind == 2) {
-      const uint32_t lo = ci == 0 ? std::max(cut, midcut) : ci == 1 ? cut : 0;
-      const uint32_t hi = ci == 0 ? UINT32_MAX : ci == 1 ? std::max(cut, midcut) : cut;
+      const uint32_t lo = ci == E_LARGE ? tier_hi : ci == E_TIER3 ? mid_hi : ci == E_MID ? cut : 0;
+      const uint32_t hi = ci == E_LARGE ? UINT32_MAX : ci == E_TIER3 ? tier_hi : ci == E_MID ? mid_hi : cut;
       gs.erase(std::remove_if(gs.begin(), gs.end(),
                               [&](uint32_t g) { return !(cfg[g]->proto.K > lo && cfg[g]->proto.K <= hi); }),
                gs.end());
-    } else if (ci == 1 || ci == 2) {
+    } else if (ci == E_TIER3 || ci == E_MID || ci == E_W8) {
       gs.clear();
-    } else if (ci >= 4 && kind == 0 && gen_cut() > 0) {
-      const bool small = ci == 5;
+    } else if (ci >= E_GEN && kind == 0 && gen_cut() > 0) {
+      const bool small = ci == E_GEN2;
       gs.erase(std::remove_if(gs.begin(), gs.end(), [&](uint32_t g) { return (cfg[g]->proto.K <= gen_cut()) != small; }),
                gs.end());
-    } else if (ci == 5) {
+    } else if (ci == E_GEN2) {
       gs.clear();
     }
     if (gs.empty()) {
       continue;
     }
-    mid_run        = mid_run || ci == 1;
+    const bool lean_run = kind == 2 && (ci == E_TIER3 || (ci == E_MID && lean_mid));
+    mid_run             = mid_run || ci == E_MID || ci == E_TIER3;
     hipStream_t st = p->s[multi_mode() == 2 ? 0 : cls_st[ci]];
     if (gated && st != p->s[0] && hipStreamWaitEvent(st, p->large_done, 0) != hipSuccess) {
       ret = SRSRAN_ERROR;
@@ -936,7 +1101,8 @@
     }
     if (gs.size() == 1) {
       const uint32_t g = gs[0];
-      ret = enqueue(cfg[g], d_input[g], in_stride[g], layout_sb, d_output[g], nof_cb[g], 0, n_end, nullptr, st);
+      ret = enqueue(cfg[g], d_input[g], in_stride[g], layout_sb, d_output[g], nof_cb[g], 0, n_end, nullptr, st,
+                    lean_run);
       continue;
     }
     const int  nsbc = cls_nsb[ci];
@@ -989,7 +1155,7 @@
       ha[k]            = a;
       hf[k]            = nblk;
       nblk += (nof_cb[g] + cpw - 1) / cpw;
-      lds = std::max(lds, kind == 2   ? (nsbc == 16  ? (w8 ? tdecs16w8::lds_bytes(a) : tdecs16::lds_bytes(a))
+      lds = std::max(lds, kind == 2   ? (nsbc == 16  ? (w8 ? tdecs16w8::lds_bytes(a) : lean_run ? tdecs16l::lds_bytes(a) : tdecs16::lds_bytes(a))
                                          : nsbc == 8 ? (w8 ? tdecs8w8::lds_bytes(a) : tdecs8::lds_bytes(a))
                                                      : tdecs1::lds_bytes(a))
                           : kind == 1 ? tdec16_lds_bytes(a)
@@ -1003,6 +1169,7 @@
     const TdecArgs* dg = reinterpret_cast<const TdecArgs*>(m.d_stage);
     const uint32_t* df = reinterpret_cast<const uint32_t*>(m.d_stage + abyte);
     if ((kind == 2   ? (nsbc == 16  ? (w8 ? tdecs16w8::multi_launch(dg, df, (int)n, nblk, lds, st)
+                                      : lean_run ? tdecs16l::multi_launch(dg, df, (int)n, nblk, lds, st)
                                           : tdecs16::multi_launch(dg, df, (int)n, nblk, lds, st))
                         : nsbc == 8 ? (w8 ? tdecs8w8::multi_launch(dg, df, (int)n, nblk, lds, st)
                                           : tdecs8::multi_launch(dg, df, (int)n, nblk, lds, st))
@@ -1023,7 +1190,8 @@
 int srsran_tdec_gpu_debug_set_stamps(void* d_buf)
 {
   using namespace srsran_amd;
-  return tdecs16::set_stamps(d_buf) == hipSuccess && tdecs8::set_stamps(d_buf) == hipSuccess &&
+  return tdecs16::set_stamps(d_buf) == hipSuccess && tdecs16l::set_stamps(d_buf) == hipSuccess &&
+                 tdecs8::set_stamps(d_buf) == hipSuccess &&
                  tdecs16w8::set_stamps(d_buf) == hipSuccess && tdecs8w8::set_stamps(d_buf) == hipSuccess
              ? SRSRAN_SUCCESS
              : SRSRAN_ERROR;
diff --git a/srsran_4g_amd/csrc/tdec_kernel.h b/srsran_4g_amd/csrc/tdec_kernel.h
--- a/srsran_4g_amd/csrc/tdec_kernel.h
+++ b/srsran_4g_amd/csrc/tdec_kernel.h
@@ -78,12 +78,16 @@
 SRSRAN_TDECS_API(tdecs16w8)
 SRSRAN_TDECS_API(tdecs8w8)
 SRSRAN_TDECS_API(tdecs1)
+SRSRAN_TDECS_API(tdecs16l)
 #undef SRSRAN_TDECS_API
+namespace tdecs16l { int occupancy(size_t lds); }
+bool tdec_lean_single(uint32_t K, uint32_t ncb);
 #ifdef TDECS_STAMPS
 namespace tdecs16 { hipError_t set_stamps(void* d_buf); }
 namespace tdecs8 { hipError_t set_stamps(void* d_buf); }
 namespace tdecs16w8 { hipError_t set_stamps(void* d_buf); }
 namespace tdecs8w8 { hipError_t set_stamps(void* d_buf); }
+namespace tdecs16l { hipError_t set_stamps(void* d_buf); }
 #endif
 bool       tdec8s_eligible(int nsb, const TdecArgs& a);
 bool       tdec1s_eligible(int nsb, const TdecArgs& a);
diff --git a/srsran_4g_amd/csrc/tdec_kernel.hip b/srsran_4g_amd/csrc/tdec_kernel.hip
--- a/srsran_4g_amd/csrc/tdec_kernel.hip
+++ b/srsran_4g_amd/csrc/tdec_kernel.hip
@@ -730,8 +730,13 @@
     return hipSuccess;
   }
   if (tdec16_eligible(nsb, a)) {
-    return tdec16_choice(a.ncb) == 2 ? (a.K <= tdecs_w8_max_k() ? tdecs16w8::launch(a, stream) : tdecs16::launch(a, stream))
-                                     : tdec16_launch(a, stream);
+    if (tdec16_choice(a.ncb) != 2) {
+      return tdec16_launch(a, stream);
+    }
+    if (a.K <= tdecs_w8_max_k()) {
+      return tdecs16w8::launch(a, stream);
+    }
+    return !a.cbs && tdec_lean_single(a.K, a.ncb) ? tdecs16l::launch(a, stream) : tdecs16::launch(a, stream);
   }
   if (tdec8s_eligible(nsb, a)) {
     return a.K <= tdecs_w8_max_k() ? tdecs8w8::launch(a, stream) : tdecs8::launch(a, stream);
diff --git a/srsran_4g_amd/csrc/tdecs_kernel.hip b/srsran_4g_amd/csrc/tdecs_kernel.hip
--- a/srsran_4g_amd/csrc/tdecs_kernel.hip
+++ b/srsran_4g_amd/csrc/tdecs_kernel.hip
@@ -11,7 +11,14 @@
 #ifndef TDECS_W
 #define TDECS_W 16
 #endif
-#if TDECS_NSB == 16 && TDECS_W == 16
+#if defined(TDECS_LEAN) && TDECS_NSB == 16 && TDECS_W == 16
+#define TDECS_NS tdecs16l
+#define TDECS_K(n) tdec16sl_##n
+#define TDECS_NAME "tdec16sl_"
+#define TDECS_WAVES 2
+#elif defined(TDECS_LEAN)
+#error "TDECS_LEAN is the 16-sub-block, 16-step kernel only"
+#elif TDECS_NSB == 16 && TDECS_W == 16
 #define TDECS_NS tdecs16
 #define TDECS_K(n) tdec16s_##n
 #define TDECS_NAME "tdec16s_"
@@ -30,6 +37,9 @@
 #else
 #error "TDECS_NSB must be 16 or 8, TDECS_W 16 or 8"
 #endif
+#ifndef TDECS_WAVES
+#define TDECS_WAVES 1
+#endif
 
 namespace srsran_amd {
 namespace TDECS_NS {
@@ -208,7 +218,46 @@
   lshort    Ssb;
   uint4*    CK;
   uint32_t* BITS;
+#ifdef TDECS_LEAN
+  uint32_t smem0, cb_b, s_b, ck_b;
+  uint32_t blk_b;
+  int      nlast;
+  uint32_t wave;
+#endif
 };
+
+#ifdef TDECS_LEAN
+__device__ __forceinline__ uint32_t lean_tid(uint32_t wave)
+{
+  uint32_t z = 0;
+  asm volatile("" : "+v"(z));
+  return wave << 6 | __builtin_amdgcn_mbcnt_hi(~0u, __builtin_amdgcn_mbcnt_lo(~0u, z));
+}
+__device__ __forceinline__ void relane(Lane& c)
+{
+  const uint32_t t   = lean_tid(c.wave);
+  const uint32_t s   = t % NSB;
+  const uint32_t cbw = (t & 63) / NSB;
+  const uint32_t b   = c.smem0 + cbw * c.cb_b;
+  c.s                = (int)s;
+  c.voff             = min(cbw, (uint32_t)c.nlast) * c.blk_b + 2 * s;
+  c.S                = (lshort)(size_t)b;
+  c.Ssb              = c.S + s * (uint32_t)c.Ls;
+  c.CK               = (uint4*)(__attribute__((address_space(3))) uint4*)(size_t)(b + c.s_b);
+  c.BITS             = (uint32_t*)(__attribute__((address_space(3))) uint32_t*)(size_t)(b + c.s_b + c.ck_b);
+}
+#define TDECS_RELANE(c) relane(c)
+template <int CTRL>
+__device__ __forceinline__ v2s row_shift(v2s v)
+{
+  static_assert(NSB == 16, "a sub-block's lanes are one DPP row");
+  return u2v((uint32_t)__builtin_amdgcn_update_dpp((int)v2u(v), (int)v2u(v), CTRL, 0xf, 0xf, false));
+}
+#else
+#define TDECS_RELANE(c) \
+  do {                  \
+  } while (0)
+#endif
 
 __device__ __forceinline__ void ck_put(const Lane& c, int m, const St& p)
 {
@@ -218,6 +267,12 @@
 {
   const uint4 v = c.CK[m * NSB + c.s];
   return St{u2v(v.x), u2v(v.y), u2v(v.z), u2v(v.w)};
+}
+
+__device__ __forceinline__ uint32_t pin(uint32_t v)
+{
+  asm volatile("" : "+v"(v));
+  return v;
 }
 
 template <bool D2>
@@ -231,6 +286,17 @@
     r.a[i]    = (soff + i) & 0xff;
     r.slot[i] = (uint16_t)((c.s * 37 + t0 + i) & 511);
     r.b[i] = (poff + 3 * i) & 0xff;
+  }
+#elif defined(TDECS_LEAN)
+  const uint32_t vin = pin(c.voff), vtf = pin(2u * (uint32_t)c.s);
+#pragma unroll
+  for (int i = 0; i < W; i++) {
+    if (D2) {
+      r.slot[i] = (uint16_t)ldb(c.rtf, vtf, soff, ROWB * i);
+    } else {
+      r.a[i] = ldb(c.rin, vin, soff, ROWB * i);
+    }
+    r.b[i] = ldb(c.rin, vin, poff, ROWB * i);
   }
 #else
 #pragma unroll
@@ -243,12 +309,6 @@
     r.b[i] = ldb(c.rin, c.voff, poff, ROWB * i);
   }
 #endif
-}
-
-__device__ __forceinline__ uint32_t pin(uint32_t v)
-{
-  asm volatile("" : "+v"(v));
-  return v;
 }
 
 __device__ __forceinline__ void set_nat(const Lane& c, int n, short o)
@@ -450,6 +510,10 @@
 {
   (void)st0;
   Lane c = cin;
+#ifdef TDECS_LEAN
+  wave = (int)cin.wave;
+  relane(c);
+#else
   asm volatile("" : "+v"(c.s));
   asm volatile("" : "+v"(c.voff));
   {
@@ -457,6 +521,7 @@
     asm volatile("" : "+v"(ssb));
     c.Ssb = (lshort)(size_t)ssb;
   }
+#endif
   const int L     = c.L;
   const int Mfull = L / W;
   const int Ma    = (L + W - 1) / W;
@@ -479,12 +544,17 @@
       pp.taken(c);
     }
     TDECS_STAMP(st0 + 1);
+    TDECS_RELANE(c);
     {
       St q;
+#ifdef TDECS_LEAN
+      q = St{row_shift<0x111>(P.a), row_shift<0x111>(P.b), row_shift<0x111>(P.c), row_shift<0x111>(P.d)};
+#else
       q.a = u2v((uint32_t)__shfl_up((int)v2u(P.a), 1, NSB));
       q.b = u2v((uint32_t)__shfl_up((int)v2u(P.b), 1, NSB));
       q.c = u2v((uint32_t)__shfl_up((int)v2u(P.c), 1, NSB));
       q.d = u2v((uint32_t)__shfl_up((int)v2u(P.d), 1, NSB));
+#endif
       P   = c.s == 0 ? alpha_known() : q;
     }
 #pragma unroll 1
@@ -502,6 +572,7 @@
     TDECS_STAMP(st0 + 2);
     __syncthreads();
     TDECS_STAMP(st0 + 3);
+    TDECS_RELANE(c);
     const int tlast = (Ma - 1) * W;
 #pragma unroll 1
     for (int ma = h; ma < Mfull; ma++) {
@@ -510,6 +581,7 @@
       pp.taken(c);
     }
     if (Ma > Mfull) {
+      TDECS_RELANE(c);
       pp.template next<true>(c, 0, xw, aux);
       alpha_llr_window<D2, BITS, false>(c, P, Mfull * W, ck_get(c, Mfull), xw, aux);
     }
@@ -530,12 +602,17 @@
       pp.taken(c);
     }
     TDECS_STAMP(st0 + 1);
+    TDECS_RELANE(c);
     {
       St q;
+#ifdef TDECS_LEAN
+      q = St{row_shift<0x101>(P.a), row_shift<0x101>(P.b), row_shift<0x101>(P.c), row_shift<0x101>(P.d)};
+#else
       q.a = u2v((uint32_t)__shfl_down((int)v2u(P.a), 1, NSB));
       q.b = u2v((uint32_t)__shfl_down((int)v2u(P.b), 1, NSB));
       q.c = u2v((uint32_t)__shfl_down((int)v2u(P.c), 1, NSB));
       q.d = u2v((uint32_t)__shfl_down((int)v2u(P.d), 1, NSB));
+#endif
       if (c.s == NSB - 1) {
         const int tail = 6 * c.KP + (D2 ? 12 : 0);
         short     xt[3], yt[3];
@@ -566,6 +643,7 @@
     TDECS_STAMP(st0 + 2);
     __syncthreads();
     TDECS_STAMP(st0 + 3);
+    TDECS_RELANE(c);
 #pragma unroll 1
     for (int mb = h - 1; mb >= 0; mb--) {
       const int t0 = mb * W;
@@ -649,6 +727,16 @@
   c.CK   = reinterpret_cast<uint4*>(base + g.s_dw);
   c.BITS = base + g.s_dw + g.ck_dw;
   uint32_t* RED = c.BITS + g.bits_dw;
+#ifdef TDECS_LEAN
+  static_assert(!ES, "the lean build has the plain launches only");
+  c.smem0 = (uint32_t)(size_t)(lshort)(short*)smem;
+  c.cb_b  = 4u * (uint32_t)g.cb_dw;
+  c.s_b   = 4u * (uint32_t)g.s_dw;
+  c.ck_b  = 4u * (uint32_t)g.ck_dw;
+  c.blk_b = 2u * a.in_stride;
+  c.nlast = min(CPWG - 1, (int)a.ncb - 1 - cb0);
+  c.wave  = __builtin_amdgcn_readfirstlane(threadIdx.x >> 6);
+#endif
 
   if constexpr (ES) {
     if (live && done && t2 == 0) {
@@ -668,10 +756,20 @@
 #pragma unroll 1
   for (int hi = 0; hi < h_end; hi++) {
     const bool crc_now = ES && hi + 1 >= a.min_iters;
+#ifdef TDECS_LEAN
+    for (int i = (int)lean_tid(c.wave); i < g.bits_dw; i += NT) {
+#pragma unroll
+      for (int j = 0; j < CPWG; j++) {
+        smem[j * g.cb_dw + g.s_dw + g.ck_dw + i] = 0u;
+      }
+    }
+    __syncthreads();
+#else
     for (int i = threadIdx.x; i < CPWG * g.bits_dw; i += NT) {
       smem[(i / g.bits_dw) * g.cb_dw + g.s_dw + g.ck_dw + i % g.bits_dw] = 0u;
     }
     __syncthreads();
+#endif
     const bool    bits = ES ? crc_now : hi + 1 == h_end;
     constexpr int BM   = ES ? 2 : 1;
     if (hi & 1) {
@@ -748,6 +846,20 @@
   }
 #endif
 
+#ifdef TDECS_LEAN
+  if (h_end > 0) {
+    const uint32_t t   = lean_tid(c.wave);
+    const int      cbo = (int)((t & 63) / NSB);
+    if (cbo <= c.nlast) {
+      const uint8_t* bits = reinterpret_cast<const uint8_t*>(smem + cbo * g.cb_dw + g.s_dw + g.ck_dw);
+      uint8_t*       out  = a.out + (size_t)(cb0 + cbo) * (K / 8);
+      for (int b = (int)((t >> 6) * NSB + t % NSB); b < K / 8; b += 2 * NSB) {
+        out[b] = bits[b];
+      }
+    }
+    return;
+  }
+#endif
   if (live && !done && h_end > 0) {
     const int      cbm   = ES ? (int)a.cbs[cbl].slot : cbl;
     uint8_t*       out   = a.out + (size_t)cbm * (ES ? a.out_stride : K / 8);
@@ -762,12 +874,12 @@
 }
 
 template <bool ES>
-__global__ __launch_bounds__(128, 1) void TDECS_K(kernel)(TdecArgs a)
+__global__ __launch_bounds__(128, TDECS_WAVES) void TDECS_K(kernel)(TdecArgs a)
 {
   body<ES>(a, blockIdx.x);
 }
 
-__global__ __launch_bounds__(128, 1) void TDECS_K(multi_kernel)(const TdecArgs* __restrict__ groups,
+__global__ __launch_bounds__(128, TDECS_WAVES) void TDECS_K(multi_kernel)(const TdecArgs* __restrict__ groups,
                                                             const uint32_t* __restrict__ first, int ngroups)
 {
   if constexpr (NSB == 16 && W == 16) {
@@ -795,11 +907,31 @@
 
 int cpw() { return CPWG; }
 
+#ifdef TDECS_LEAN
+int occupancy(size_t lds)
+{
+  int n1 = 0, n2 = 0;
+  if (hipOccupancyMaxActiveBlocksPerMultiprocessor(&n1, TDECS_K(kernel)<false>, 128, lds) != hipSuccess ||
+      hipOccupancyMaxActiveBlocksPerMultiprocessor(&n2, TDECS_K(multi_kernel), 128, lds) != hipSuccess) {
+    return -1;
+  }
+  return n1 < n2 ? n1 : n2;
+}
+#endif
+
 hipError_t launch(const TdecArgs& a, hipStream_t stream)
 {
   StageScope timing_scope(ST_TDEC, stream);
   const int    grid = (a.ncb + CPWG - 1) / CPWG;
   const size_t lds  = lds_bytes(a);
+#ifdef TDECS_LEAN
+  if (a.cbs) {
+    return hipErrorInvalidValue;
+  }
+  tdec_set_last_kernel(TDECS_NAME "kernel<false>");
+  hipLaunchKernelGGL((TDECS_K(kernel)<false>), dim3(grid), dim3(128), lds, stream, a);
+  return hipGetLastError();
+#else
   tdec_set_last_kernel(a.cbs ? TDECS_NAME "kernel<true>" : TDECS_NAME "kernel<false>");
   if (a.cbs) {
     hipLaunchKernelGGL((TDECS_K(kernel)<true>), dim3(grid), dim3(128), lds, stream, a);
@@ -807,6 +939,7 @@
     hipLaunchKernelGGL((TDECS_K(kernel)<false>), dim3(grid), dim3(128), lds, stream, a);
   }
   return hipGetLastError();
+#endif
 }
 
 hipError_t multi_launch(const TdecArgs* d_groups, const uint32_t* d_first, int ngroups, uint32_t nblocks, size_t lds,
diff --git a/srsran_4g_amd/tdec.py b/srsran_4g_amd/tdec.py
--- a/srsran_4g_amd/tdec.py
+++ b/srsran_4g_amd/tdec.py
@@ -92,6 +92,10 @@
         "srsran_tdec_gpu_set_w8_fused_max_k": ([u32], None),
         "srsran_tdec_gpu_get_w8_fused_max_k": ([], u32),
         "srsran_tdec_gpu_get_generic_single_threshold": ([], u32),
+        "srsran_tdec_gpu_set_lean": ([ctypes.c_int], None),
+        "srsran_tdec_gpu_get_lean": ([], ctypes.c_int),
+        "srsran_tdec_gpu_set_lean_cuts": ([u32, u32], None),
+        "srsran_tdec_gpu_get_lean_cut": ([u32], u32),
     }
     for name, (args, res) in sig.items():
         f = getattr(lib, name)
@@ -142,6 +146,22 @@
 
     def __exit__(self, *exc):
         load_library().srsran_tdec_gpu_set_w8_fused_max_k(self.old)
+
+
+class lean(pair_threshold):
+
+    def __enter__(self):
+        lib = load_library()
+        self.old = lib.srsran_tdec_gpu_get_lean()
+        lib.srsran_tdec_gpu_set_lean(self.n)
+        return self
+
+    def __exit__(self, *exc):
+        load_library().srsran_tdec_gpu_set_lean(self.old)
+
+
+def lean_cut(nof_workgroups):
+    return load_library().srsran_tdec_gpu_get_lean_cut(nof_workgroups)
 
 
 class class_single_threshold:
```

After: 35260 Mbps. About the same (-0.2%).
